# silencht/SG-SLAM

Measured on AMD Instinct MI355X. Metric: tracked frames/sec (640x480 RGB-D), higher is better.
Workload: dtype u8/f32(bf16x3 matrix products)/f64

## Files before the change

### include/sgx_debug.h

```cpp
#ifndef SGX_DEBUG_H
#define SGX_DEBUG_H
#include "sgx.h"
#ifdef __cplusplus
extern "C" {
#endif

int sgx_orb_debug_level_geometry(const sgx_orb *h, int level, int32_t *w, int32_t *hgt, int32_t *stride);
int sgx_orb_debug_set_unfused_pyramid(int on);
int sgx_orb_debug_read_level(sgx_orb *h, int frame, int level, uint8_t *dst );
int sgx_orb_debug_read_candidates(sgx_orb *h, int frame, int level, int32_t *x, int32_t *y, int32_t *score, int cap, int *n);
int sgx_debug_flow_affine_batch_dev(int batch, int cap, const sgx_keypoint *d_keys, const int32_t *d_n, const float *d_A, const float *d_shift, const float *d_boxes,
                                    int max_boxes, float *d_prev_xy, void *stream);
int sgx_pose_opt_debug_set_threads(int threads_per_frame);
int sgx_ba_debug_last_plan(int32_t plan[4]);
int sgx_ba_debug_set_init(int mode);
int sgx_ba_debug_set_jobs(int host);
int sgx_ba_debug_set_solver(int mode);
int sgx_det_debug_read_blob(sgx_det *h, const char *blob_name, int image, float *dst, int cap, int *n);
int sgx_flow_debug_read_level(sgx_flow *h, int slot, int frame, int level, uint8_t *img);
int sgx_flow_debug_level_size(const sgx_flow *h, int level, int32_t *w, int32_t *hgt);
int sgx_pnp_debug_betas(int which, const double *L, const double *rho, double *betas);
int sgx_debug_corun_bf16(int blocks, int iters, int launches, void *stream);
int sgx_det_debug_detection_output(sgx_det *h, const float *loc, const float *conf, int batch, sgx_det_result *results);
int sgx_det_debug_continued(sgx_det *h, int *count);
int sgx_det_debug_set_fusion(int on);
int sgx_det_debug_set_irb(int on);
int sgx_det_debug_set_block_fusion(int on);
int sgx_det_debug_set_gemm(int mode);
int sgx_det_debug_set_legacy_kernels(int on);
int sgx_det_debug_time_ops(sgx_det *h, const uint8_t *d_img, int pitch, int batch, int reps, float *ms, int cap, int *nops);
int sgx_det_debug_run_step(sgx_det *h, const uint8_t *d_img, int pitch, int batch, int step, int reps, void *stream);
int sgx_orb_debug_run_octree(sgx_orb *h, int level, const uint32_t *packed, int n, uint32_t *out_sel, int cap, int *nsel);

#ifdef __cplusplus
}
#endif
#endif
```

### sg_slam_amd/capi.py

```python
import ctypes as C
import numpy as np

KP_DTYPE = np.dtype([('x', 'f4'), ('y', 'f4'), ('size', 'f4'), ('angle', 'f4'), ('response', 'f4'),
                     ('octave', 'i4'), ('class_id', 'i4')])


class SgxError(RuntimeError):
    pass


class Camera(C.Structure):
    _fields_ = [('fx', C.c_float), ('fy', C.c_float), ('cx', C.c_float), ('cy', C.c_float), ('bf', C.c_float),
                ('min_x', C.c_float), ('max_x', C.c_float), ('min_y', C.c_float), ('max_y', C.c_float)]


class BaProblem(C.Structure):
    _fields_ = [('n_poses', C.c_int32), ('n_points', C.c_int32), ('n_edges', C.c_int32), ('poses', C.c_void_p), ('pose_fixed', C.c_void_p),
                ('points', C.c_void_p), ('edge_pose', C.c_void_p), ('edge_point', C.c_void_p), ('edge_obs', C.c_void_p), ('edge_info', C.c_void_p)]


class BaStats(C.Structure):
    _fields_ = [('iterations_first', C.c_int32), ('iterations_second', C.c_int32), ('free_poses', C.c_int32), ('reserved', C.c_int32),
                ('chi2_first', C.c_double), ('chi2_second', C.c_double)]


SGX_DET_MAX = 100


class Detection(C.Structure):
    _fields_ = [(k, C.c_float) for k in ('label', 'score', 'xmin', 'ymin', 'xmax', 'ymax')]


class Object2D(C.Structure):
    _fields_ = [('id', C.c_int32)] + [(k, C.c_float) for k in ('prob', 'x', 'y', 'w', 'h')]


class DetResult(C.Structure):
    _fields_ = [('n_raw', C.c_int32), ('raw', Detection * SGX_DET_MAX), ('n_objects', C.c_int32), ('objects', Object2D * SGX_DET_MAX),
                ('have_dynamic_for_mapping', C.c_int32), ('have_dynamic_for_rm_feature', C.c_int32),
                ('n_map_boxes', C.c_int32), ('map_boxes', Object2D * SGX_DET_MAX), ('n_rm_boxes', C.c_int32), ('rm_boxes', Object2D * SGX_DET_MAX)]


class FlowConfig(C.Structure):
    _fields_ = [('width', C.c_int32), ('height', C.c_int32), ('max_batch', C.c_int32), ('win_size', C.c_int32), ('max_level', C.c_int32),
                ('max_count', C.c_int32), ('epsilon', C.c_double)]


class TrackerConfig(C.Structure):
    _fields_ = [('streams', C.c_int32), ('width', C.c_int32), ('height', C.c_int32), ('nfeatures', C.c_int32), ('scale_factor', C.c_float), ('nlevels', C.c_int32),
                ('ini_th_fast', C.c_int32), ('min_th_fast', C.c_int32), ('cam', Camera), ('depth_map_factor', C.c_float), ('th_projection', C.c_float),
                ('local_map', C.c_int32), ('dynamic_mask', C.c_int32), ('max_boxes', C.c_int32), ('pipelined', C.c_int32)]


class OrbConfig(C.Structure):
    _fields_ = [('nfeatures', C.c_int32), ('scale_factor', C.c_float), ('nlevels', C.c_int32),
                ('ini_th_fast', C.c_int32), ('min_th_fast', C.c_int32), ('width', C.c_int32),
                ('height', C.c_int32), ('max_batch', C.c_int32)]


SYMBOLS = [
    'sgx_version', 'sgx_status_string', 'sgx_orb_create', 'sgx_orb_destroy', 'sgx_orb_keypoint_capacity', 'sgx_orb_get_tables',
    'sgx_orb_extract_batch_dev', 'sgx_orb_extract', 'sgx_orb_last_status', 'sgx_profile_enable', 'sgx_profile_num_classes', 'sgx_profile_class_name',
    'sgx_profile_read', 'sgx_match_project_frame_batch_dev', 'sgx_match_project_frame', 'sgx_match_project_local_batch_dev',
    'sgx_match_project_local', 'sgx_frame_stereo_from_rgbd_batch_dev', 'sgx_frame_unproject_batch_dev', 'sgx_frame_make_map_points_batch_dev',
    'sgx_frame_merge_matches_batch_dev', 'sgx_pose_optimization_batch_dev', 'sgx_pose_optimization', 'sgx_frame_motion_model_batch_dev',
    'sgx_local_bundle_adjustment', 'sgx_bundle_adjustment', 'sgx_det_create', 'sgx_det_destroy', 'sgx_det_info', 'sgx_det_detect',
    'sgx_det_detect_batch_dev', 'sgx_det_forward_batch_dev', 'sgx_frame_compact_keys_batch_dev', 'sgx_frame_gray_from_color_batch_dev',
    'sgx_det_gemm_mode', 'sgx_det_plan_step', 'sgx_dynamic_mask_batch_dev', 'sgx_tracker_create', 'sgx_tracker_destroy',
    'sgx_tracker_keypoint_capacity', 'sgx_tracker_record_bytes', 'sgx_tracker_set_initial_pose', 'sgx_tracker_step_dev', 'sgx_tracker_host_buffers',
    'sgx_tracker_step_host', 'sgx_tracker_wait_inputs', 'sgx_tracker_sync', 'sgx_tracker_read', 'sgx_tracker_snapshot_pose_dev',
    'sgx_tracker_snapshot_boxes_dev', 'sgx_tracker_pack_records_dev', 'sgx_tracker_frame_dev', 'sgx_tracker_extractor', 'sgx_flow_create',
    'sgx_dist_unique_id', 'sgx_dist_create', 'sgx_dist_destroy', 'sgx_dist_world', 'sgx_dist_gather_records',
    'sgx_flow_destroy', 'sgx_flow_reset', 'sgx_flow_levels', 'sgx_flow_lk_batch_dev', 'sgx_flow_lk', 'sgx_fundamental_ransac_batch_dev',
    'sgx_find_fundamental_mat', 'sgx_hamming_matrix', 'sgx_hamming_matrix_dev', 'sgx_match_search_for_triangulation', 'sgx_match_search_by_bow',
    'sgx_match_search_by_bow_kf', 'sgx_match_fuse_search', 'sgx_match_project_keyframe', 'sgx_match_fuse_search_sim3',
    'sgx_triangulate_new_map_points', 'sgx_mappoint_update_normal_and_depth', 'sgx_mappoint_distinctive_descriptors', 'sgx_sim3_solver_create',
    'sgx_sim3_solver_set_ransac_parameters', 'sgx_sim3_solver_iterate', 'sgx_sim3_solver_get_estimate', 'sgx_sim3_solver_destroy',
    'sgx_match_search_for_initialization', 'sgx_voc_load', 'sgx_voc_create', 'sgx_voc_info', 'sgx_voc_destroy', 'sgx_voc_transform',
    'sgx_voc_transform_batch_dev', 'sgx_voc_score', 'sgx_match_project_sim3', 'sgx_match_search_by_sim3', 'sgx_optimize_sim3',
    'sgx_optimize_essential_graph', 'sgx_correct_map_points', 'sgx_undistort_points', 'sgx_frame_undistort_stereo_rgbd_batch_dev', 'sgx_frame_image_bounds',
    'sgx_tracker_set_distortion', 'sgx_tracker_frame_keys_un_dev', 'sgx_pnp_solver_create', 'sgx_pnp_solver_set_ransac_parameters', 'sgx_pnp_solver_iterate',
    'sgx_pnp_solver_get_estimate', 'sgx_pnp_solver_destroy', 'sgx_pnp_batch_create', 'sgx_pnp_batch_set_dev', 'sgx_pnp_batch_iterate_dev', 'sgx_pnp_batch_destroy',
]
TAP_SYMBOLS = [
    'sgx_orb_debug_level_geometry', 'sgx_orb_debug_set_unfused_pyramid', 'sgx_orb_debug_read_level', 'sgx_orb_debug_read_candidates',
    'sgx_orb_debug_run_octree', 'sgx_pose_opt_debug_set_threads', 'sgx_ba_debug_set_solver', 'sgx_ba_debug_set_jobs', 'sgx_ba_debug_set_init', 'sgx_ba_debug_last_plan', 'sgx_det_debug_read_blob',
    'sgx_det_debug_detection_output', 'sgx_det_debug_continued', 'sgx_debug_flow_affine_batch_dev', 'sgx_det_debug_set_fusion', 'sgx_det_debug_set_legacy_kernels',
    'sgx_det_debug_set_block_fusion', 'sgx_det_debug_set_irb', 'sgx_det_debug_set_gemm', 'sgx_det_debug_time_ops', 'sgx_det_debug_run_step', 'sgx_flow_debug_read_level',
    'sgx_flow_debug_level_size', 'sgx_debug_corun_bf16', 'sgx_pnp_debug_betas',
]


def _vp(x):
    if x is None:
        return None
    if isinstance(x, int):
        return C.c_void_p(x)
    if hasattr(x, 'data_ptr'):
        return C.c_void_p(x.data_ptr())
    return x.ctypes.data_as(C.c_void_p)


class SgxLib:
    def __init__(self, path):
        self.path = path
        self.dll = C.CDLL(path)
        d = self.dll
        d.sgx_version.restype = C.c_char_p
        d.sgx_status_string.restype = C.c_char_p
        d.sgx_status_string.argtypes = [C.c_int]
        d.sgx_orb_create.argtypes = [C.POINTER(OrbConfig), C.POINTER(C.c_void_p)]
        d.sgx_orb_destroy.argtypes = [C.c_void_p]
        d.sgx_orb_destroy.restype = None
        d.sgx_orb_keypoint_capacity.argtypes = [C.c_void_p]
        d.sgx_orb_get_tables.argtypes = [C.c_void_p] + [C.c_void_p] * 5
        d.sgx_orb_extract_batch_dev.argtypes = [C.c_void_p, C.c_void_p, C.c_int, C.c_int, C.c_void_p, C.c_void_p,
                                                C.c_void_p, C.c_int, C.c_void_p]
        d.sgx_orb_extract.argtypes = [C.c_void_p, C.c_void_p, C.c_int, C.c_void_p, C.c_void_p, C.c_int, C.POINTER(C.c_int)]
        d.sgx_orb_last_status.argtypes = [C.c_void_p, C.c_void_p]

        d.sgx_profile_enable.argtypes = [C.c_int]
        d.sgx_profile_class_name.restype = C.c_char_p
        d.sgx_profile_class_name.argtypes = [C.c_int]
        d.sgx_profile_read.argtypes = [C.c_void_p, C.c_void_p, C.c_int]

        vp = C.c_void_p
        d.sgx_match_project_frame_batch_dev.argtypes = [C.c_int, C.c_int] + [vp] * 13 + [C.POINTER(Camera), vp, C.c_int, C.c_float, C.c_int, C.c_int, vp, vp, vp]
        d.sgx_match_project_frame.argtypes = [C.c_int] + [vp] * 4 + [C.c_int] + [vp] * 7 + [C.POINTER(Camera), vp, C.c_int, C.c_float, C.c_int, C.c_int, vp, vp]
        d.sgx_frame_stereo_from_rgbd_batch_dev.argtypes = [C.c_int, C.c_int, vp, vp, vp, C.c_int, C.c_int, C.c_float, C.c_float, vp, vp, vp]
        d.sgx_frame_unproject_batch_dev.argtypes = [C.c_int, C.c_int, vp, vp, vp, vp, C.POINTER(Camera), vp, vp, vp]
        d.sgx_pose_optimization_batch_dev.argtypes = [C.c_int, C.c_int, vp, vp, vp, vp, vp, vp, C.c_int, vp, C.c_int, C.POINTER(Camera), vp, vp, vp, vp]
        d.sgx_pose_optimization.argtypes = [C.c_int, vp, vp, vp, vp, vp, C.c_int, C.POINTER(Camera), vp, vp, vp]
        d.sgx_frame_motion_model_batch_dev.argtypes = [C.c_int, vp, vp, vp, vp, vp]
        d.sgx_local_bundle_adjustment.argtypes = [C.POINTER(BaProblem), C.POINTER(Camera), vp, vp, C.POINTER(BaStats)]
        d.sgx_bundle_adjustment.argtypes = [C.POINTER(BaProblem), C.POINTER(Camera), C.c_int, vp, C.c_int, C.POINTER(BaStats)]
        d.sgx_det_create.argtypes = [C.c_char_p, vp, C.c_size_t, C.c_int, C.c_int, C.c_int, C.c_float, C.c_float, C.POINTER(vp)]
        d.sgx_det_destroy.argtypes = [vp]; d.sgx_det_destroy.restype = None
        d.sgx_det_info.argtypes = [vp, C.POINTER(C.c_int32), C.POINTER(C.c_int32), C.POINTER(C.c_int32), C.POINTER(C.c_double)]
        d.sgx_det_detect.argtypes = [vp, vp, C.c_int, C.c_int, C.POINTER(DetResult)]
        d.sgx_det_detect_batch_dev.argtypes = [vp, vp, C.c_int, C.c_int, vp, vp, vp, C.c_int, vp, vp]
        d.sgx_det_forward_batch_dev.argtypes = [vp, vp, C.c_int, C.c_int, C.POINTER(vp), C.POINTER(vp), vp]
        d.sgx_det_gemm_mode.argtypes = [vp]
        d.sgx_tracker_create.argtypes = [C.POINTER(TrackerConfig), vp, C.POINTER(vp)]
        d.sgx_tracker_destroy.argtypes = [vp]; d.sgx_tracker_destroy.restype = None
        d.sgx_tracker_keypoint_capacity.argtypes = [vp]
        d.sgx_tracker_record_bytes.argtypes = [vp]
        d.sgx_tracker_set_initial_pose.argtypes = [vp, vp]
        d.sgx_tracker_step_dev.argtypes = [vp, vp, C.c_int, vp, vp, C.c_int, vp]
        d.sgx_tracker_host_buffers.argtypes = [vp, C.c_int, C.POINTER(vp), C.POINTER(C.c_int), C.POINTER(vp)]
        d.sgx_tracker_step_host.argtypes = [vp, C.c_int, C.c_int]
        d.sgx_tracker_sync.argtypes = [vp]
        d.sgx_tracker_wait_inputs.argtypes = [vp, C.c_int]
        d.sgx_tracker_read.argtypes = [vp] * 10
        d.sgx_tracker_snapshot_pose_dev.argtypes = [vp, vp]
        d.sgx_tracker_snapshot_boxes_dev.argtypes = [vp, C.c_int, vp, vp]
        d.sgx_tracker_pack_records_dev.argtypes = [vp, vp, vp]
        d.sgx_dist_unique_id.argtypes = [vp]
        d.sgx_dist_create.argtypes = [vp, C.c_int, C.c_int, C.POINTER(vp)]
        d.sgx_dist_destroy.argtypes = [vp]; d.sgx_dist_destroy.restype = None
        d.sgx_dist_world.argtypes = [vp, C.POINTER(C.c_int32), C.POINTER(C.c_int32)]
        d.sgx_dist_gather_records.argtypes = [vp, vp, C.c_size_t, vp, C.c_int, vp]
        d.sgx_tracker_frame_dev.argtypes = [vp] + [C.POINTER(vp)] * 6
        d.sgx_tracker_extractor.argtypes = [vp]; d.sgx_tracker_extractor.restype = vp
        d.sgx_det_plan_step.argtypes = [vp, C.c_int, C.c_char_p, C.c_int]
        d.sgx_dynamic_mask_batch_dev.argtypes = [C.c_int, C.c_int, vp, vp, vp, vp, vp, vp, C.c_int, vp, vp]
        d.sgx_frame_gray_from_color_batch_dev.argtypes = [C.c_int, C.c_int, C.c_int, vp, C.c_int, C.c_int, C.c_int, vp, C.c_int, vp]
        d.sgx_frame_compact_keys_batch_dev.argtypes = [C.c_int, C.c_int, vp, vp, vp, vp, vp, C.c_int, vp, vp, vp, vp]
        d.sgx_match_project_local.argtypes = [C.c_int] + [vp] * 5 + [C.c_int] + [vp] * 7 + [C.POINTER(Camera), vp, C.c_int, C.c_float, C.c_float, C.c_float, C.c_float, vp, vp, vp]
        d.sgx_match_project_local_batch_dev.argtypes = [C.c_int, C.c_int] + [vp] * 6 + [C.c_int] + [vp] * 8 + [C.POINTER(Camera), vp, C.c_int, C.c_float, C.c_float, C.c_float, C.c_float, vp, vp, vp, vp]
        d.sgx_undistort_points.argtypes = [C.c_int, vp, vp, vp, C.c_int, vp]
        d.sgx_frame_undistort_stereo_rgbd_batch_dev.argtypes = [C.c_int, C.c_int, vp, vp, vp, C.c_int, C.POINTER(Camera), vp, C.c_int, C.c_int, C.c_float, vp, vp, vp, vp]
        d.sgx_frame_image_bounds.argtypes = [C.c_int, C.c_int, vp, vp, C.c_int, C.POINTER(Camera)]
        d.sgx_tracker_set_distortion.argtypes = [vp, vp, C.c_int, C.POINTER(Camera)]
        d.sgx_tracker_frame_keys_un_dev.argtypes = [vp, C.POINTER(vp)]
        d.sgx_frame_make_map_points_batch_dev.argtypes = [C.c_int, C.c_int, C.c_int] + [vp] * 7 + [C.c_int] + [vp] * 7
        d.sgx_frame_merge_matches_batch_dev.argtypes = [C.c_int, C.c_int] + [vp] * 10
        d.sgx_flow_create.argtypes = [C.POINTER(FlowConfig), C.POINTER(vp)]
        d.sgx_flow_destroy.argtypes = [vp]; d.sgx_flow_destroy.restype = None
        d.sgx_flow_reset.argtypes = [vp]
        d.sgx_flow_levels.argtypes = [vp]
        d.sgx_flow_lk_batch_dev.argtypes = [vp, vp, C.c_int, C.c_int, vp, vp, C.c_int, vp, vp, C.POINTER(C.c_int32), vp]
        d.sgx_flow_lk.argtypes = [vp, vp, vp, C.c_int, vp, C.c_int, vp, vp]
        d.sgx_fundamental_ransac_batch_dev.argtypes = [C.c_int, C.c_int] + [vp] * 6 + [C.c_int, C.c_double, C.c_double, vp, vp, vp, vp]
        d.sgx_find_fundamental_mat.argtypes = [vp, vp, C.c_int, C.c_double, C.c_double, vp, vp, vp]
        d.sgx_hamming_matrix.argtypes = [vp, C.c_int, vp, C.c_int, vp]
        d.sgx_optimize_essential_graph.argtypes = [C.c_int, vp, vp, C.c_int, vp, vp, vp, C.c_int, C.c_int, vp, vp]
        d.sgx_correct_map_points.argtypes = [C.c_int, vp, vp, C.c_int, vp, vp, vp]
        d.sgx_optimize_sim3.argtypes = [C.c_int] + [vp] * 9 + [C.c_float, C.c_int, vp, vp, vp]
        d.sgx_match_project_keyframe.argtypes = [C.c_int] + [vp] * 4 + [C.c_int] + [vp] * 6 + [C.POINTER(Camera), vp, C.c_int, C.c_float, C.c_float, C.c_int, C.c_int, vp, vp]
        d.sgx_match_search_by_bow.argtypes = [C.c_int] + [vp] * 4 + [C.c_int] + [vp] * 3 + [C.c_float, C.c_int, vp, vp]
        d.sgx_match_fuse_search_sim3.argtypes = [C.c_int, vp, vp, vp, C.c_int] + [vp] * 6 + [vp, vp, C.c_int, C.c_float, C.c_float, vp, vp, vp]
        d.sgx_match_project_sim3.argtypes = [C.c_int, vp, vp, vp, vp, C.c_int] + [vp] * 6 + [vp, vp, C.c_int, C.c_float, C.c_int, vp, vp]
        d.sgx_match_search_by_sim3.argtypes = ([C.c_int] + [vp] * 8) * 2 + [vp, vp, C.c_int, C.c_float, C.c_float, vp, vp, C.c_float, vp, vp]
        d.sgx_match_search_for_initialization.argtypes = [C.c_int, vp, vp, C.c_int, vp, vp, vp, C.c_int, C.c_float, C.c_int, vp, vp, vp]
        d.sgx_sim3_solver_create.argtypes = [C.c_int] + [vp] * 6 + [C.c_int, C.c_uint, vp]
        d.sgx_sim3_solver_set_ransac_parameters.argtypes = [vp, C.c_double, C.c_int, C.c_int]
        d.sgx_sim3_solver_iterate.argtypes = [vp, C.c_int] + [vp] * 7
        d.sgx_sim3_solver_get_estimate.argtypes = [vp] * 5
        d.sgx_sim3_solver_destroy.argtypes = [vp]; d.sgx_sim3_solver_destroy.restype = None
        d.sgx_pnp_solver_create.argtypes = [C.c_int] + [vp] * 4 + [C.c_uint, vp]
        d.sgx_pnp_solver_set_ransac_parameters.argtypes = [vp, C.c_double, C.c_int, C.c_int, C.c_int, C.c_float, C.c_float]
        d.sgx_pnp_solver_iterate.argtypes = [vp, C.c_int] + [vp] * 7
        d.sgx_pnp_solver_get_estimate.argtypes = [vp] * 6
        d.sgx_pnp_solver_destroy.argtypes = [vp]; d.sgx_pnp_solver_destroy.restype = None
        d.sgx_pnp_batch_create.argtypes = [C.c_int, C.c_int, vp]
        d.sgx_pnp_batch_set_dev.argtypes = [vp, C.c_int] + [vp] * 8
        d.sgx_pnp_batch_iterate_dev.argtypes = [vp, C.c_int, vp, C.c_int, vp, vp, vp, vp]
        d.sgx_pnp_batch_destroy.argtypes = [vp]; d.sgx_pnp_batch_destroy.restype = None
        d.sgx_mappoint_update_normal_and_depth.argtypes = [C.c_int] + [vp] * 6 + [C.c_int, vp, vp, vp]
        d.sgx_mappoint_distinctive_descriptors.argtypes = [C.c_int, vp, vp, vp, vp]
        d.sgx_triangulate_new_map_points.argtypes = [C.c_int, vp] + [C.c_int] + [vp] * 5 + [C.c_int] + [vp] * 5 + [vp, vp, vp, C.c_int, vp, vp, vp]
        d.sgx_voc_load.argtypes = [C.c_char_p, vp]
        d.sgx_voc_create.argtypes = [C.c_int] * 5 + [vp] * 5
        d.sgx_voc_info.argtypes = [vp] * 7
        d.sgx_voc_destroy.argtypes = [vp]; d.sgx_voc_destroy.restype = None
        d.sgx_voc_transform.argtypes = [vp, C.c_int, vp, C.c_int, vp, vp, vp, vp, vp]
        d.sgx_voc_transform_batch_dev.argtypes = [vp, vp, C.c_size_t, vp, C.c_int, C.c_int, C.c_int, vp, vp, vp, vp]
        d.sgx_voc_score.argtypes = [vp, C.c_int, vp, vp, C.c_int, vp, vp, vp]
        d.sgx_match_search_by_bow_kf.argtypes = [C.c_int] + [vp] * 4 + [C.c_int] + [vp] * 4 + [C.c_float, C.c_int, vp, vp]
        d.sgx_match_fuse_search.argtypes = [C.c_int] + [vp] * 4 + [C.c_int] + [vp] * 6 + [C.POINTER(Camera), vp, vp, C.c_int, C.c_float, C.c_float, vp, vp, vp]
        d.sgx_hamming_matrix_dev.argtypes = [vp, C.c_int, vp, C.c_int, vp, vp]
        d.sgx_match_search_for_triangulation.argtypes = [C.c_int] + [vp] * 6 + [C.c_int] + [vp] * 6 + [vp, C.POINTER(Camera), vp, vp, C.c_int, C.c_int, C.c_int, vp, vp]

        self.has_taps = hasattr(d, 'sgx_det_debug_read_blob')
        if self.has_taps:
            d.sgx_orb_debug_level_geometry.argtypes = [C.c_void_p, C.c_int] + [C.POINTER(C.c_int32)] * 3
            d.sgx_orb_debug_read_level.argtypes = [C.c_void_p, C.c_int, C.c_int, C.c_void_p]
            d.sgx_orb_debug_read_candidates.argtypes = [C.c_void_p, C.c_int, C.c_int, C.c_void_p, C.c_void_p, C.c_void_p, C.c_int, C.POINTER(C.c_int)]
            d.sgx_orb_debug_run_octree.argtypes = [C.c_void_p, C.c_int, C.c_void_p, C.c_int, C.c_void_p, C.c_int, C.POINTER(C.c_int)]
            d.sgx_orb_debug_set_unfused_pyramid.argtypes = [C.c_int]
            d.sgx_pose_opt_debug_set_threads.argtypes = [C.c_int]
            d.sgx_ba_debug_set_solver.argtypes = [C.c_int]
            d.sgx_ba_debug_set_jobs.argtypes = [C.c_int]
            d.sgx_ba_debug_set_init.argtypes = [C.c_int]
            d.sgx_ba_debug_last_plan.argtypes = [C.c_void_p]
            d.sgx_det_debug_detection_output.argtypes = [vp, vp, vp, C.c_int, C.POINTER(DetResult)]
            d.sgx_det_debug_continued.argtypes = [vp, C.POINTER(C.c_int)]
            d.sgx_det_debug_read_blob.argtypes = [vp, C.c_char_p, C.c_int, vp, C.c_int, C.POINTER(C.c_int)]
            for nm in ('fusion', 'legacy_kernels', 'block_fusion', 'irb', 'gemm'):
                getattr(d, 'sgx_det_debug_set_' + nm).argtypes = [C.c_int]
            d.sgx_det_debug_time_ops.argtypes = [vp, vp, C.c_int, C.c_int, C.c_int, vp, C.c_int, C.POINTER(C.c_int)]
            d.sgx_det_debug_run_step.argtypes = [vp, vp, C.c_int, C.c_int, C.c_int, C.c_int, vp]
            d.sgx_debug_flow_affine_batch_dev.argtypes = [C.c_int, C.c_int, vp, vp, vp, vp, vp, C.c_int, vp, vp]
            d.sgx_flow_debug_read_level.argtypes = [vp, C.c_int, C.c_int, C.c_int, vp]
            d.sgx_debug_corun_bf16.argtypes = [C.c_int, C.c_int, C.c_int, vp]
            d.sgx_pnp_debug_betas.argtypes = [C.c_int, vp, vp, vp]
            d.sgx_flow_debug_level_size.argtypes = [vp, C.c_int, C.POINTER(C.c_int32), C.POINTER(C.c_int32)]

    def tap(self, name):
        if not self.has_taps:
            raise SgxError(f'{name}: {self.path} is the product build and has no test taps; use tests/taps/libsgx_taps.so (make -C sg_slam_amd/csrc taps)')
        return getattr(self.dll, name)

    def version(self):
        return self.dll.sgx_version().decode()

    def check(self, rc, what=''):
        if rc != 0:
            raise SgxError(f'{what}: {self.dll.sgx_status_string(rc).decode()} ({rc})')

    def profile_enable(self, on=True):
        self.check(self.dll.sgx_profile_enable(int(on)))

    def profile_read(self, reset=True):
        n = self.dll.sgx_profile_num_classes()
        ms = np.zeros(n, 'f4'); cnt = np.zeros(n, 'i4')
        self.check(self.dll.sgx_profile_read(_vp(ms), _vp(cnt), int(reset)), 'sgx_profile_read')
        return {self.dll.sgx_profile_class_name(k).decode(): (float(ms[k]), int(cnt[k])) for k in range(n)}
```

### sg_slam_amd/csrc/sgx_flow.cpp

```cpp
#include "sgx_flow_kernels.h"
#include "sgx_prof.h"
#include "sgx_stage.h"
#include "../../include/sgx.h"
#ifdef SGX_DEBUG_TAPS
#include "../../include/sgx_debug.h"
#endif
#include <stdio.h>
#include <stdlib.h>
#include <string.h>
#include <new>
#include <vector>


struct sgx_flow {
    sgx_flow_config cfg;
    SgxLkGeom g;
    uint8_t *img[2] = { nullptr, nullptr };
    int cur = 0;
    int prev_batch = 0;
};

extern "C" int sgx_flow_create(const sgx_flow_config *cfg, sgx_flow **out)
{
    if (!cfg || !out) return SGX_ERR_INVALID;
    *out = nullptr;
    if (cfg->width < 1 || cfg->height < 1 || cfg->max_batch < 1 || cfg->max_count < 0 || !(cfg->epsilon >= 0)) return SGX_ERR_INVALID;
    if (cfg->win_size != SGX_LK_WIN || cfg->max_level < 0 || cfg->max_level >= SGX_LK_MAXL) return SGX_ERR_UNSUPPORTED;
    if (cfg->width <= 1 || cfg->height <= 1) return SGX_ERR_UNSUPPORTED;
    { const unsigned long long qw = (unsigned long long)((cfg->width + 3) >> 2); if (qw * qw * (unsigned long long)cfg->height >= (1ull << 32)) return SGX_ERR_UNSUPPORTED; }
    sgx_flow *h = new (std::nothrow) sgx_flow();
    if (!h) return SGX_ERR_NOMEM;
    h->cfg = *cfg;
    SgxLkGeom &g = h->g;
    memset(&g, 0, sizeof g);
    int w = cfg->width, hh = cfg->height; unsigned io = 0;
    for (int l = 0;; l++) {
        g.w[l] = w; g.h[l] = hh; g.pitch[l] = (w + 3) & ~3; g.ioff[l] = io;
        io += (unsigned)g.pitch[l] * (unsigned)hh;
        g.nl = l + 1;
        if (l == cfg->max_level) break;
        const int nw = (w + 1) / 2, nh = (hh + 1) / 2;
        if (nw <= cfg->win_size || nh <= cfg->win_size) break;
        w = nw; hh = nh;
    }
    g.img_stride = (io + 15u + 64u) & ~15u;
    for (int s = 0; s < 2; s++)
        if (hipMalloc((void **)&h->img[s], (size_t)g.img_stride * cfg->max_batch) != hipSuccess) { sgx_flow_destroy(h); return SGX_ERR_NOMEM; }
    *out = h;
    return SGX_OK;
}

extern "C" void sgx_flow_destroy(sgx_flow *h)
{
    if (!h) return;
    for (int s = 0; s < 2; s++) if (h->img[s]) (void)hipFree(h->img[s]);
    delete h;
}

extern "C" int sgx_flow_reset(sgx_flow *h) { if (!h) return SGX_ERR_INVALID; h->prev_batch = 0; return SGX_OK; }
extern "C" int sgx_flow_levels(const sgx_flow *h) { return h ? h->g.nl : SGX_ERR_INVALID; }

static int build_pyramid(sgx_flow *h, int slot, const uint8_t *d_gray, int pitch, int batch, sgx_stream_t st)
{
    const SgxLkGeom &g = h->g;
    uint8_t *base = h->img[slot];
    sgx_prof_begin(SGX_K_LK_PYR, st);
    auto magic = [](int d) -> unsigned { return d <= 1 ? 0u : (unsigned)((0x100000000ull + (unsigned)d - 1) / (unsigned)d); };
    SGX_LAUNCH(k_lk_copy, dim3(((g.pitch[0] >> 2) * g.h[0] + 255) / 256, batch), dim3(256), st, d_gray, g.w[0], g.h[0], pitch, base, g.pitch[0], g.img_stride, magic(g.pitch[0] >> 2));
    for (int l = 1; l < g.nl; l++)
        SGX_LAUNCH(k_lk_pyrdown, dim3(((g.pitch[l] >> 2) * g.h[l] + 255) / 256, batch), dim3(256), st, (const uint8_t *)(base + g.ioff[l - 1]), g.w[l - 1], g.h[l - 1], g.pitch[l - 1],
                   g.img_stride, base + g.ioff[l], g.w[l], g.h[l], g.pitch[l], g.img_stride, magic(g.pitch[l] >> 2));
    sgx_prof_end(SGX_K_LK_PYR, st);
    SGX_CHECK_HIP(hipGetLastError());
    return SGX_OK;
}

static int track(sgx_flow *h, int cur_slot, int prev_slot, int batch, const sgx_keypoint *d_keys, const int32_t *d_n, int cap, float *d_prev_xy, uint8_t *d_status, sgx_stream_t st)
{
    SgxLkArgs A;
    A.cur_img = h->img[cur_slot]; A.prev_img = h->img[prev_slot];
    A.keys = (const uint8_t *)d_keys; A.n = d_n; A.cap = cap; A.prev_xy = d_prev_xy; A.status = d_status;
    A.max_count = h->cfg.max_count > 100 ? 100 : h->cfg.max_count;
    double eps = h->cfg.epsilon > 10. ? 10. : h->cfg.epsilon;
    A.eps2 = eps * eps; A.min_eig = (float)1e-4;
    sgx_prof_begin(SGX_K_LK_TRACK, st);
    static const int kpw = sgx_getenv("SGX_LK_KPW") ? atoi(sgx_getenv("SGX_LK_KPW")) : 2;
    A.batch = batch; A.kblocks = (cap + 4 * kpw - 1) / (4 * kpw);
#ifdef SGX_DEBUG_TAPS
    if (kpw == 4) { auto kfn = k_lk_trackN<4>; SGX_LAUNCH(kfn, dim3((unsigned)A.kblocks * (unsigned)batch), dim3(256), st, h->g, A); }
    else if (kpw != 2) { A.kblocks = (cap + 3) / 4; SGX_LAUNCH(k_lk_track, dim3((unsigned)A.kblocks * (unsigned)batch), dim3(256), st, h->g, A); }
    else
#endif
    { auto kfn = k_lk_trackN<2>; SGX_LAUNCH(kfn, dim3((unsigned)A.kblocks * (unsigned)batch), dim3(256), st, h->g, A); }
    sgx_prof_end(SGX_K_LK_TRACK, st);
    SGX_CHECK_HIP(hipGetLastError());
    return SGX_OK;
}

extern "C" int sgx_flow_lk_batch_dev(sgx_flow *h, const uint8_t *d_gray, int pitch, int batch, const sgx_keypoint *d_keys, const int32_t *d_n, int cap,
                                     float *d_prev_xy, uint8_t *d_status, int32_t *have_prev, void *stream)
{
    if (!h || !d_gray || batch < 1 || batch > h->cfg.max_batch || pitch < h->cfg.width) return SGX_ERR_INVALID;
    if ((pitch & 3) || ((uintptr_t)d_gray & 3)) return SGX_ERR_INVALID;
    sgx_stream_t st = (sgx_stream_t)stream;
    const int cur = h->cur, prev = cur ^ 1;
    const bool tracked = h->prev_batch == batch;
    if (tracked && (!d_keys || !d_n || !d_prev_xy || cap < 1)) return SGX_ERR_INVALID;
    int rc = build_pyramid(h, cur, d_gray, pitch, batch, st);
    if (rc != SGX_OK) return rc;
    if (tracked) { rc = track(h, cur, prev, batch, d_keys, d_n, cap, d_prev_xy, d_status, st); if (rc != SGX_OK) return rc; }
    if (have_prev) *have_prev = tracked ? 1 : 0;
    h->cur = prev; h->prev_batch = batch;
    return SGX_OK;
}

extern "C" int sgx_flow_lk(sgx_flow *h, const uint8_t *gray_from, const uint8_t *gray_to, int stride, const float *pts, int n, float *next_pts, uint8_t *status)
{
    if (!h || !gray_from || !gray_to || stride < h->cfg.width || n < 0 || (n > 0 && (!pts || !next_pts))) return SGX_ERR_INVALID;
    if (n == 0) return SGX_OK;
    const int W = h->cfg.width, H = h->cfg.height, P = (W + 3) & ~3;
    std::vector<uint8_t> pack((size_t)P * H * 2, 0);
    for (int y = 0; y < H; y++) { memcpy(&pack[(size_t)y * P], gray_to + (size_t)y * stride, (size_t)W); memcpy(&pack[(size_t)(H + y) * P], gray_from + (size_t)y * stride, (size_t)W); }
    std::vector<sgx_keypoint> kp((size_t)n);
    for (int i = 0; i < n; i++) { memset(&kp[(size_t)i], 0, sizeof(sgx_keypoint)); kp[(size_t)i].x = pts[2 * i]; kp[(size_t)i].y = pts[2 * i + 1]; }
    SgxStaged dI, dK, dN, dO, dS;
    int rc;
    if ((rc = dI.put(0, pack.data(), pack.size())) != SGX_OK || (rc = dK.put(1, kp.data(), kp.size() * sizeof(sgx_keypoint))) != SGX_OK ||
        (rc = dN.put(2, &n, sizeof n)) != SGX_OK || (rc = dO.put(3, nullptr, (size_t)n * 8)) != SGX_OK || (rc = dS.put(4, nullptr, (size_t)n)) != SGX_OK) return rc;
    const int keep_cur = h->cur, keep_prev = h->prev_batch;
    if ((rc = build_pyramid(h, 1, (const uint8_t *)dI.p, P, 1, 0)) != SGX_OK) return rc;
    if ((rc = build_pyramid(h, 0, (const uint8_t *)dI.p + (size_t)P * H, P, 1, 0)) != SGX_OK) return rc;
    if ((rc = track(h, 0, 1, 1, (const sgx_keypoint *)dK.p, (const int32_t *)dN.p, n, (float *)dO.p, (uint8_t *)dS.p, 0)) != SGX_OK) return rc;
    SGX_CHECK_HIP(hipMemcpy(next_pts, dO.p, (size_t)n * 8, hipMemcpyDeviceToHost));
    if (status) SGX_CHECK_HIP(hipMemcpy(status, dS.p, (size_t)n, hipMemcpyDeviceToHost));
    h->cur = keep_cur; h->prev_batch = 0; (void)keep_prev;
    return SGX_OK;
}

SGX_TAP int sgx_flow_debug_read_level(sgx_flow *h, int slot, int frame, int level, uint8_t *img )
{
    if (!h || slot < 0 || slot > 1 || frame < 0 || frame >= h->cfg.max_batch || level < 0 || level >= h->g.nl) return SGX_ERR_INVALID;
    const SgxLkGeom &g = h->g;
    SGX_CHECK_HIP(hipDeviceSynchronize());
    if (!img) return SGX_ERR_INVALID;
    {
        std::vector<uint8_t> t((size_t)g.pitch[level] * g.h[level]);
        SGX_CHECK_HIP(hipMemcpy(t.data(), h->img[slot] + (size_t)frame * g.img_stride + g.ioff[level], t.size(), hipMemcpyDeviceToHost));
        for (int y = 0; y < g.h[level]; y++) memcpy(img + (size_t)y * g.w[level], &t[(size_t)y * g.pitch[level]], (size_t)g.w[level]);
    }
    return SGX_OK;
}
SGX_TAP int sgx_flow_debug_level_size(const sgx_flow *h, int level, int32_t *w, int32_t *hh)
{
    if (!h || level < 0 || level >= h->g.nl || !w || !hh) return SGX_ERR_INVALID;
    *w = h->g.w[level]; *hh = h->g.h[level];
    return SGX_OK;
}

#if defined(SGX_DEBUG_TAPS) && !defined(SGX_EMU)
typedef float sgx_dbg_f16v __attribute__((ext_vector_type(16)));
typedef __bf16 sgx_dbg_bf8 __attribute__((ext_vector_type(8)));
SGX_KERNEL_OCC(256, 2) k_dbg_corun_bf16(float *o, int iters)
{
    const uint32_t x = threadIdx.x * 2654435761u + blockIdx.x, y = x ^ 0x9e3779b9u;
    sgx_dbg_f16v acc = {0}; sgx_dbg_bf8 a, b;
    for (int i = 0; i < 8; i++) { a[i] = (__bf16)(float)((x >> i) & 7); b[i] = (__bf16)(float)((y >> i) & 3); }
    for (int i = 0; i < iters; i++) acc = __builtin_amdgcn_mfma_f32_32x32x16_bf16(a, b, acc, 0, 0, 0);
    float s = 0.f; for (int i = 0; i < 16; i++) s += acc[i];
    o[(blockIdx.x & 1023) * 256 + threadIdx.x] = s;
}
#endif
SGX_TAP int sgx_debug_corun_bf16(int blocks, int iters, int launches, void *stream)
{
#if defined(SGX_DEBUG_TAPS) && !defined(SGX_EMU)
    static float *sink = nullptr;
    if (blocks < 1 || iters < 1 || launches < 1) return SGX_ERR_INVALID;
    if (!sink) SGX_CHECK_HIP(hipMalloc((void **)&sink, 1024 * 256 * sizeof(float)));
    for (int l = 0; l < launches; l++) SGX_LAUNCH(k_dbg_corun_bf16, dim3((unsigned)blocks), dim3(256), (sgx_stream_t)stream, sink, iters);
    SGX_CHECK_HIP(hipGetLastError());
    return SGX_OK;
#else
    (void)blocks; (void)iters; (void)launches; (void)stream;
    return SGX_ERR_UNSUPPORTED;
#endif
}

extern "C" int sgx_fundamental_ransac_batch_dev(int batch, int cap, const sgx_keypoint *d_keys, const int32_t *d_n, const float *d_prev_xy,
                                                const int32_t *d_pre_have_dynamic, const float *d_pre_boxes, const int32_t *d_pre_nboxes, int max_boxes,
                                                double threshold, double confidence, double *d_F, int32_t *d_ok, int32_t *d_stats, void *stream)
{
    if (batch < 1 || cap < 1 || !d_keys || !d_n || !d_prev_xy || !d_F || !d_ok || max_boxes < 0) return SGX_ERR_INVALID;
    if (cap > SGX_FM_MAXPTS) return SGX_ERR_UNSUPPORTED;
    SgxFmArgs A;
    A.keys = (const uint8_t *)d_keys; A.n = d_n; A.cap = cap; A.prev_xy = d_prev_xy;
    A.pre_have = d_pre_have_dynamic; A.pre_boxes = d_pre_boxes; A.pre_nboxes = d_pre_nboxes; A.max_boxes = max_boxes;
    if (threshold <= 0) threshold = 3;
    if (confidence < DBL_EPSILON || confidence > 1 - DBL_EPSILON) confidence = 0.99;
    A.threshold = threshold; A.confidence = confidence; A.max_iters = 1000;
    A.F = d_F; A.ok = d_ok; A.stats = d_stats;
    const size_t lds = (size_t)cap * 16 + 1024 + (((size_t)cap + 15) & ~(size_t)15);
    sgx_prof_begin(SGX_K_FM_RANSAC, (sgx_stream_t)stream);
    SGX_LAUNCH_DYN(k_fm_ransac, dim3(batch), dim3(256), lds, (sgx_stream_t)stream, A);
    sgx_prof_end(SGX_K_FM_RANSAC, (sgx_stream_t)stream);
    SGX_CHECK_HIP(hipGetLastError());
    return SGX_OK;
}

extern "C" int sgx_find_fundamental_mat(const float *pts1, const float *pts2, int n, double threshold, double confidence, double *F, int32_t *ok, int32_t *stats)
{
    if (n < 0 || (n > 0 && (!pts1 || !pts2)) || !F || !ok) return SGX_ERR_INVALID;
    if (n > SGX_FM_MAXPTS) return SGX_ERR_UNSUPPORTED;
    const int cap = n > 0 ? n : 1;
    std::vector<sgx_keypoint> kp((size_t)cap);
    memset(kp.data(), 0, kp.size() * sizeof(sgx_keypoint));
    for (int i = 0; i < n; i++) { kp[(size_t)i].x = pts1[2 * i]; kp[(size_t)i].y = pts1[2 * i + 1]; }
    SgxStaged dK, dN, dP, dF, dO, dS;
    int rc;
    if ((rc = dK.put(0, kp.data(), kp.size() * sizeof(sgx_keypoint))) != SGX_OK || (rc = dN.put(1, &n, sizeof n)) != SGX_OK ||
        (rc = dP.put(2, n ? pts2 : nullptr, (size_t)cap * 8)) != SGX_OK || (rc = dF.put(3, nullptr, 72)) != SGX_OK || (rc = dO.put(4, nullptr, 4)) != SGX_OK ||
        (rc = dS.put(5, nullptr, 16)) != SGX_OK) return rc;
    rc = sgx_fundamental_ransac_batch_dev(1, cap, (const sgx_keypoint *)dK.p, (const int32_t *)dN.p, (const float *)dP.p, nullptr, nullptr, nullptr, 0, threshold, confidence,
                                          (double *)dF.p, (int32_t *)dO.p, (int32_t *)dS.p, nullptr);
    if (rc != SGX_OK) return rc;
    SGX_CHECK_HIP(hipMemcpy(F, dF.p, 72, hipMemcpyDeviceToHost));
    SGX_CHECK_HIP(hipMemcpy(ok, dO.p, 4, hipMemcpyDeviceToHost));
    if (stats) SGX_CHECK_HIP(hipMemcpy(stats, dS.p, 16, hipMemcpyDeviceToHost));
    return SGX_OK;
}
```

### sg_slam_amd/csrc/sgx_flow_kernels.h

```cpp
#pragma once
#include "sgx_rt.h"
#include "sgx_block.h"
#include <float.h>
#include <math.h>

#define SGX_LK_MAXL 4
#define SGX_LK_WIN 21
#define SGX_LK_TILE_PITCH 36
struct SgxLkGeom {
    int nl;
    int w[SGX_LK_MAXL], h[SGX_LK_MAXL], pitch[SGX_LK_MAXL];
    unsigned ioff[SGX_LK_MAXL];
    unsigned img_stride;
};

SGX_DEV int sgx_reflect101(int p, int len)
{
    if (len == 1) return 0;
    while (p < 0 || p >= len) { if (p < 0) p = -p; else p = 2 * len - 2 - p; }
    return p;
}
SGX_DEV int sgx_floor_f(float v) { return (int)floorf(v); }
SGX_DEV float sgx_i64_to_f32(long long v)
{
    const long long hi = v >> 24; const int lo = (int)(v - (hi << 24));
    return (float)(int)hi * 16777216.0f + (float)lo;
}

SGX_DEV unsigned sgx_lk_udiv(unsigned n, unsigned m)
{
#ifndef SGX_EMU
    return m ? __umulhi(n, m) : n;
#else
    return m ? (unsigned)(((unsigned long long)n * m) >> 32) : n;
#endif
}
SGX_KERNEL(256) k_lk_copy(const uint8_t *src, int w, int h, int spitch, uint8_t *dst, int dpitch, unsigned dstride, unsigned qw_magic)
{
    SGX_THREADS_BEGIN(tid)
    const int f = (int)blockIdx.y, qw = dpitch >> 2, q = (int)blockIdx.x * 256 + tid;
    if (q < qw * h) {
        const int y = (int)sgx_lk_udiv((unsigned)q, qw_magic), x = (q - y * qw) * 4;
        const uint8_t *s = src + ((size_t)f * h + y) * spitch;
        uint32_t v;
        if (x + 4 <= w) v = *(const uint32_t *)(s + x);
        else { v = 0; for (int i = 0; x + i < w; i++) v |= (uint32_t)s[x + i] << (8 * i); }
        *(uint32_t *)(dst + (size_t)f * dstride + (size_t)y * dpitch + x) = v;
    }
    SGX_THREADS_END
}

SGX_KERNEL(256) k_lk_pyrdown(const uint8_t *src, int sw, int sh, int spitch, unsigned sstride, uint8_t *dst, int dw, int dh, int dpitch, unsigned dstride, unsigned qw_magic)
{
    SGX_THREADS_BEGIN(tid)
    const int f = (int)blockIdx.y, qw = dpitch >> 2, q = (int)blockIdx.x * 256 + tid;
    if (q < qw * dh) {
        const int y = (int)sgx_lk_udiv((unsigned)q, qw_magic), X = (q - y * qw) * 4;
        const uint8_t *S = src + (size_t)f * sstride;
        int acc[4] = { 0, 0, 0, 0 };
        const bool fast = X >= 2 && 2 * X + 11 < spitch && 2 * X + 8 <= sw - 1;
#pragma unroll
        for (int k = 0; k < 5; k++) {
            const int wk = k == 0 || k == 4 ? 1 : k == 2 ? 6 : 4;
            const uint8_t *row = S + (size_t)sgx_reflect101(2 * y - 2 + k, sh) * spitch;
            int p[11];
            if (fast) {
                const uint32_t *r4 = (const uint32_t *)(row + 2 * X - 4);
                const uint32_t a = r4[0], b = r4[1], c = r4[2], d = r4[3];
                p[0] = (a >> 16) & 255; p[1] = a >> 24;
                p[2] = b & 255; p[3] = (b >> 8) & 255; p[4] = (b >> 16) & 255; p[5] = b >> 24;
                p[6] = c & 255; p[7] = (c >> 8) & 255; p[8] = (c >> 16) & 255; p[9] = c >> 24;
                p[10] = d & 255;
            } else {
#pragma unroll
                for (int i = 0; i < 11; i++) p[i] = row[sgx_reflect101(2 * X - 2 + i, sw)];
            }
#pragma unroll
            for (int o = 0; o < 4; o++) acc[o] += wk * (p[2 * o + 2] * 6 + (p[2 * o + 1] + p[2 * o + 3]) * 4 + p[2 * o] + p[2 * o + 4]);
        }
        uint32_t out = 0;
#pragma unroll
        for (int o = 0; o < 4; o++) out |= (uint32_t)((acc[o] + 128) >> 8) << (8 * o);
        *(uint32_t *)(dst + (size_t)f * dstride + (size_t)y * dpitch + X) = out;
    }
    SGX_THREADS_END
}

struct SgxLkWeights { int w00, w01, w10, w11; };
SGX_DEV SgxLkWeights sgx_lk_weights(float a, float b)
{
    SgxLkWeights k;
    k.w00 = sgx_cvround((1.f - a) * (1.f - b) * (float)(1 << 14));
    k.w01 = sgx_cvround(a * (1.f - b) * (float)(1 << 14));
    k.w10 = sgx_cvround((1.f - a) * b * (float)(1 << 14));
    k.w11 = (1 << 14) - k.w00 - k.w01 - k.w10;
    return k;
}
#define SGX_LK_DESCALE(x, n) (((x) + (1 << ((n) - 1))) >> (n))

struct SgxLkStep { float dx, dy; };
SGX_DEV SgxLkStep sgx_lk_step(float A11, float A12, float A22, float D, long long sb1, long long sb2)
{
    const float FLT_SCALE = 1.f / (1 << 20);
    const float b1 = sgx_i64_to_f32(sb1) * FLT_SCALE, b2 = sgx_i64_to_f32(sb2) * FLT_SCALE;
    SgxLkStep s;
    s.dx = (A12 * b2 - A22 * b1) * D;
    s.dy = (A12 * b1 - A11 * b2) * D;
    return s;
}

struct SgxLkArgs {
    const uint8_t *cur_img, *prev_img;
    const uint8_t *keys; const int *n; int cap;
    float *prev_xy; uint8_t *status;
    int max_count; double eps2; float min_eig;
    int batch, kblocks;
};
SGX_DEV void sgx_lk_decode_block(int i, int batch, int kblocks, int &f, int &kb)
{
    const int full = (batch / 8) * 8;
    if (i < full * kblocks) { const int x = i & 7, j = i >> 3; kb = j % kblocks; f = x + 8 * (j / kblocks); }
    else { const int j = i - full * kblocks; f = full + j / kblocks; kb = j % kblocks; }
}

#ifdef SGX_EMU
static inline int sgx_lk_px(const uint8_t *I, int w, int h, int pitch, int x, int y) { return I[(size_t)sgx_reflect101(y, h) * pitch + sgx_reflect101(x, w)]; }
static void sgx_lk_track_point(const SgxLkGeom &g, const uint8_t *I0, const uint8_t *J0, float kx, float ky, int max_count, double eps2, float min_eig,
                               float *ox, float *oy, uint8_t *ost)
{
    const int W = SGX_LK_WIN; const float half = (W - 1) * 0.5f, FLT_SCALE = 1.f / (1 << 20);
    float outx = 0.f, outy = 0.f; uint8_t status = 1;
    static thread_local short Iw[SGX_LK_WIN * SGX_LK_WIN], dIw[SGX_LK_WIN * SGX_LK_WIN * 2];
    for (int level = g.nl - 1; level >= 0; level--) {
        const int w = g.w[level], h = g.h[level], pitch = g.pitch[level];
        const uint8_t *I = I0 + g.ioff[level], *J = J0 + g.ioff[level];
        const float sc = 1.0f / (float)(1 << level);
        float prevx = kx * sc, prevy = ky * sc, nextx, nexty;
        if (level == g.nl - 1) { nextx = prevx; nexty = prevy; } else { nextx = outx * 2.f; nexty = outy * 2.f; }
        outx = nextx; outy = nexty;
        prevx -= half; prevy -= half;
        const int ipx = sgx_floor_f(prevx), ipy = sgx_floor_f(prevy);
        if (ipx < -W || ipx >= w || ipy < -W || ipy >= h) { if (level == 0) status = 0; continue; }
        SgxLkWeights k = sgx_lk_weights(prevx - ipx, prevy - ipy);
        long long s11 = 0, s12 = 0, s22 = 0;
        for (int y = 0; y < W; y++) for (int x = 0; x < W; x++) {
            int pv[4], dx[4], dy[4];
            for (int c = 0; c < 4; c++) {
                const int gx = ipx + x + (c & 1), gy = ipy + y + (c >> 1);
                pv[c] = sgx_lk_px(I, w, h, pitch, gx, gy);
                if (gx < 0 || gy < 0 || gx >= w || gy >= h) { dx[c] = dy[c] = 0; }
                else {
                    int t0[3], t1[3];
                    for (int q = 0; q < 3; q++) {
                        const int a = sgx_lk_px(I, w, h, pitch, gx - 1 + q, gy - 1), b = sgx_lk_px(I, w, h, pitch, gx - 1 + q, gy), cc = sgx_lk_px(I, w, h, pitch, gx - 1 + q, gy + 1);
                        t0[q] = (a + cc) * 3 + b * 10; t1[q] = cc - a;
                    }
                    dx[c] = t0[2] - t0[0]; dy[c] = (t1[0] + t1[2]) * 3 + t1[1] * 10;
                }
            }
            const int iv = SGX_LK_DESCALE(pv[0] * k.w00 + pv[1] * k.w01 + pv[2] * k.w10 + pv[3] * k.w11, 9);
            const int ix = SGX_LK_DESCALE(dx[0] * k.w00 + dx[1] * k.w01 + dx[2] * k.w10 + dx[3] * k.w11, 14);
            const int iy = SGX_LK_DESCALE(dy[0] * k.w00 + dy[1] * k.w01 + dy[2] * k.w10 + dy[3] * k.w11, 14);
            Iw[y * W + x] = (short)iv; dIw[(y * W + x) * 2] = (short)ix; dIw[(y * W + x) * 2 + 1] = (short)iy;
            s11 += (long long)ix * ix; s12 += (long long)ix * iy; s22 += (long long)iy * iy;
        }
        const float A11 = sgx_i64_to_f32(s11) * FLT_SCALE, A12 = sgx_i64_to_f32(s12) * FLT_SCALE, A22 = sgx_i64_to_f32(s22) * FLT_SCALE;
        float D = A11 * A22 - A12 * A12;
        const float minEig = (A22 + A11 - sqrtf((A11 - A22) * (A11 - A22) + 4.f * A12 * A12)) / (float)(2 * W * W);
        if (minEig < min_eig || D < FLT_EPSILON) { if (level == 0) status = 0; continue; }
        D = 1.f / D;
        nextx -= half; nexty -= half;
        float pdx = 0.f, pdy = 0.f;
        for (int j = 0; j < max_count; j++) {
            const int inx = sgx_floor_f(nextx), iny = sgx_floor_f(nexty);
            if (inx < -W || inx >= w || iny < -W || iny >= h) { if (level == 0) status = 0; break; }
            k = sgx_lk_weights(nextx - inx, nexty - iny);
            long long sb1 = 0, sb2 = 0;
            for (int y = 0; y < W; y++) for (int x = 0; x < W; x++) {
                int pv[4];
                for (int c = 0; c < 4; c++) pv[c] = sgx_lk_px(J, w, h, pitch, inx + x + (c & 1), iny + y + (c >> 1));
                const int diff = SGX_LK_DESCALE(pv[0] * k.w00 + pv[1] * k.w01 + pv[2] * k.w10 + pv[3] * k.w11, 9) - Iw[y * W + x];
                sb1 += (long long)diff * dIw[(y * W + x) * 2]; sb2 += (long long)diff * dIw[(y * W + x) * 2 + 1];
            }
            const SgxLkStep st = sgx_lk_step(A11, A12, A22, D, sb1, sb2);
            nextx += st.dx; nexty += st.dy;
            outx = nextx + half; outy = nexty + half;
            if ((double)st.dx * st.dx + (double)st.dy * st.dy <= eps2) break;
            if (j > 0 && fabs((double)(st.dx + pdx)) < 0.01 && fabs((double)(st.dy + pdy)) < 0.01) { outx -= st.dx * 0.5f; outy -= st.dy * 0.5f; break; }
            pdx = st.dx; pdy = st.dy;
        }
        if (status && level == 0) {
            const int ix = sgx_floor_f(outx - half), iy = sgx_floor_f(outy - half);
            if (ix < -W || ix >= w || iy < -W || iy >= h) status = 0;
        }
    }
    *ox = outx; *oy = outy; *ost = status;
}
SGX_KERNEL(256) k_lk_track(SgxLkGeom g, SgxLkArgs A)
{
    SGX_THREADS_BEGIN(tid)
    int f, kb;
    sgx_lk_decode_block((int)blockIdx.x, A.batch, A.kblocks, f, kb);
    const int kp = kb * 4 + (tid >> 6);
    if ((tid & 63) == 0 && kp < A.n[f] && kp < A.cap) {
        const float *kpt = (const float *)(A.keys + ((size_t)f * A.cap + kp) * 28);
        float ox, oy; uint8_t st;
        sgx_lk_track_point(g, A.cur_img + (size_t)f * g.img_stride, A.prev_img + (size_t)f * g.img_stride, kpt[0], kpt[1], A.max_count, A.eps2, A.min_eig, &ox, &oy, &st);
        A.prev_xy[2 * ((size_t)f * A.cap + kp)] = ox; A.prev_xy[2 * ((size_t)f * A.cap + kp) + 1] = oy;
        if (A.status) A.status[(size_t)f * A.cap + kp] = st;
    }
    SGX_THREADS_END
}
#else
SGX_DEV int sgx_wave_sum_i32(int v)
{
    v += __builtin_amdgcn_update_dpp(0, v, 0xB1, 0xF, 0xF, true);
    v += __builtin_amdgcn_update_dpp(0, v, 0x4E, 0xF, 0xF, true);
    v += __builtin_amdgcn_update_dpp(0, v, 0x124, 0xF, 0xF, true);
    v += __builtin_amdgcn_update_dpp(0, v, 0x128, 0xF, 0xF, true);
    v += __builtin_amdgcn_update_dpp(0, v, 0x142, 0xA, 0xF, false);
    v += __builtin_amdgcn_update_dpp(0, v, 0x143, 0xC, 0xF, false);
    return __builtin_amdgcn_readlane(v, 63);
}
SGX_DEV float sgx_wave_sum_f32(int v)
{
    const int lo = sgx_wave_sum_i32(v & 0xFFFF), hi = sgx_wave_sum_i32(v >> 16);
    return fmaf((float)hi, 65536.0f, (float)lo);
}
SGX_DEV int sgx_mul24(int a, int b) { return __mul24(a, b); }
SGX_DEV int sgx_reflect1(int p, int len) { p = p < 0 ? -p : p; p = p >= len ? 2 * len - 2 - p : p; return min(max(p, 0), len - 1); }

typedef short sgx_i16x2 __attribute__((ext_vector_type(2)));
typedef unsigned short sgx_u16x2 __attribute__((ext_vector_type(2)));
SGX_DEV sgx_i16x2 sgx_as_i16x2(uint32_t v) { return __builtin_bit_cast(sgx_i16x2, v); }
SGX_DEV uint32_t sgx_as_u32(sgx_i16x2 v) { return __builtin_bit_cast(uint32_t, v); }
#define SGX_LK_PAIR(hi, lo, a, b) sgx_as_i16x2(__builtin_amdgcn_perm((hi), (lo), (uint32_t)(a) | 0x0c00u | ((uint32_t)(b) << 16) | 0x0c000000u))
SGX_DEV sgx_i16x2 sgx_lk_next(sgx_i16x2 p, sgx_i16x2 q) { return sgx_as_i16x2(__builtin_amdgcn_alignbit(sgx_as_u32(q), sgx_as_u32(p), 16)); }
#if defined(SGX_LK_NODOT) && !defined(SGX_EMU)
SGX_DEV int sgx_lk_dot2_mad(sgx_i16x2 a, sgx_i16x2 b, int c)
{
    const uint32_t ua = __builtin_bit_cast(uint32_t, a), ub = __builtin_bit_cast(uint32_t, b);
    asm("v_mad_i32_i16 %0, %1, %2, %0 op_sel:[0,0,0,0]" : "+v"(c) : "v"(ua), "v"(ub));
    asm("v_mad_i32_i16 %0, %1, %2, %0 op_sel:[1,1,0,0]" : "+v"(c) : "v"(ua), "v"(ub));
    return c;
}
#define SGX_LK_DOT2(a, b, c) sgx_lk_dot2_mad((a), (b), (c))
#else
#define SGX_LK_DOT2(a, b, c) __builtin_amdgcn_sdot2((a), (b), (c), false)
#endif
SGX_DEV int sgx_lk_dot2_keep(sgx_i16x2 a, sgx_i16x2 b, int c) { return SGX_LK_DOT2(a, b, c); }

template <int PASSES>
SGX_DEV void sgx_lk_stage(uint32_t *tile, const uint8_t *img, int w, int h, int pitch, int ox, int oy, int rl, int cl)
{
    __builtin_amdgcn_fence(__ATOMIC_SEQ_CST, "wavefront"); __builtin_amdgcn_wave_barrier();
    const int gx = ox + 4 * cl;
    const bool inside = gx >= 0 && gx + 4 <= w;
    if (rl < 7) {
        uint32_t v[PASSES];
        if (inside) {
#pragma unroll
            for (int p = 0; p < PASSES; p++) v[p] = *(const uint32_t *)(img + (size_t)sgx_reflect1(oy + p * 7 + rl, h) * pitch + gx);
        } else {
            const int x0 = sgx_reflect1(gx, w), x1 = sgx_reflect1(gx + 1, w), x2 = sgx_reflect1(gx + 2, w), x3 = sgx_reflect1(gx + 3, w);
#pragma unroll
            for (int p = 0; p < PASSES; p++) {
                const uint8_t *src = img + (size_t)sgx_reflect1(oy + p * 7 + rl, h) * pitch;
                v[p] = (uint32_t)src[x0] | ((uint32_t)src[x1] << 8) | ((uint32_t)src[x2] << 16) | ((uint32_t)src[x3] << 24);
            }
        }
#pragma unroll
        for (int p = 0; p < PASSES; p++) tile[(p * 7 + rl) * (SGX_LK_TILE_PITCH / 4) + cl] = v[p];
    }
    __builtin_amdgcn_fence(__ATOMIC_SEQ_CST, "wavefront"); __builtin_amdgcn_wave_barrier();
}

#ifdef SGX_DEBUG_TAPS
SGX_KERNEL(256) k_lk_track(SgxLkGeom g, SgxLkArgs A)
{
    __shared__ uint32_t tiles[4][35 * SGX_LK_TILE_PITCH / 4 + 5];
    const int tid = (int)threadIdx.x, lane = tid & 63, wv = tid >> 6;
    int f, kb;
    sgx_lk_decode_block((int)blockIdx.x, A.batch, A.kblocks, f, kb);
    const int kp = kb * 4 + wv;
    if (kp >= A.n[f] || kp >= A.cap) return;
    uint32_t *tile = tiles[wv];
    const uint8_t *tile8 = (const uint8_t *)tile;
    const int W = SGX_LK_WIN; const float half = 10.0f, FLT_SCALE = 1.f / (1 << 20);
    const float *kpt = (const float *)(A.keys + ((size_t)f * A.cap + kp) * 28);
    const float kx = __builtin_bit_cast(float, __builtin_amdgcn_readfirstlane(__builtin_bit_cast(int, kpt[0])));
    const float ky = __builtin_bit_cast(float, __builtin_amdgcn_readfirstlane(__builtin_bit_cast(int, kpt[1])));
    const uint8_t *I0 = A.cur_img + (size_t)f * g.img_stride, *J0 = A.prev_img + (size_t)f * g.img_stride;
    const int r = lane / 3, s7 = (lane - 3 * r) * 7;
    const int rl = lane / 9, cl = lane - 9 * rl;
    const bool active = lane < 63;
    const int lane_off = active ? r * SGX_LK_TILE_PITCH + s7 : 0;
    float outx = 0.f, outy = 0.f; int status = 1;

    for (int level = g.nl - 1; level >= 0; level--) {
        const int w = g.w[level], h = g.h[level], pitch = g.pitch[level];
        const uint8_t *I = I0 + g.ioff[level], *J = J0 + g.ioff[level];
        const float sc = 1.0f / (float)(1 << level);
        float prevx = kx * sc, prevy = ky * sc, nextx, nexty;
        if (level == g.nl - 1) { nextx = prevx; nexty = prevy; } else { nextx = outx * 2.f; nexty = outy * 2.f; }
        outx = nextx; outy = nexty;
        prevx -= half; prevy -= half;
        const int ipx = sgx_floor_f(prevx), ipy = sgx_floor_f(prevy);
        if (ipx < -W || ipx >= w || ipy < -W || ipy >= h) { if (level == 0) status = 0; continue; }
        SgxLkWeights k = sgx_lk_weights(prevx - ipx, prevy - ipy);
        sgx_i16x2 W0 = sgx_as_i16x2((uint32_t)k.w00 | ((uint32_t)k.w01 << 16)), W1 = sgx_as_i16x2((uint32_t)k.w10 | ((uint32_t)k.w11 << 16));

        int ivb[7]; int ix[7], iy[7];
        int s11 = 0, s12 = 0, s22 = 0;
        {
            const int gy0 = ipy + r, gx0 = ipx + s7;
            sgx_i16x2 P[4][5];
            const bool direct = ipx >= 1 && ipx + 25 < w && ipy >= 1 && ipy + 22 < h;
            if (direct) {
                const uint8_t *gb = I + (size_t)(active ? gy0 - 1 : ipy) * pitch + (active ? gx0 - 1 : ipx);
#pragma unroll
                for (int j = 0; j < 4; j++) {
                    uint32_t q[3];
                    __builtin_memcpy(q, gb + (size_t)j * pitch, 12);
                    P[j][0] = SGX_LK_PAIR(q[0], q[0], 0, 1); P[j][1] = SGX_LK_PAIR(q[0], q[0], 2, 3);
                    P[j][2] = SGX_LK_PAIR(q[1], q[1], 0, 1); P[j][3] = SGX_LK_PAIR(q[1], q[1], 2, 3);
                    P[j][4] = SGX_LK_PAIR(q[2], q[2], 0, 1);
                }
            } else {
                const int tx = ((ipx - 1) >> 2) << 2, ty = ipy - 1;
                sgx_lk_stage<4>(tile, I, w, h, pitch, tx, ty, rl, cl);
                const uint8_t *tb = tile8 + lane_off + (ipx - 1 - tx);
#pragma unroll
                for (int j = 0; j < 4; j++) {
                    uint32_t q[3];
                    __builtin_memcpy(q, tb + j * SGX_LK_TILE_PITCH, 12);
                    P[j][0] = SGX_LK_PAIR(q[0], q[0], 0, 1); P[j][1] = SGX_LK_PAIR(q[0], q[0], 2, 3);
                    P[j][2] = SGX_LK_PAIR(q[1], q[1], 0, 1); P[j][3] = SGX_LK_PAIR(q[1], q[1], 2, 3);
                    P[j][4] = SGX_LK_PAIR(q[2], q[2], 0, 1);
                }
            }
            const sgx_i16x2 c3 = { 3, 3 }, c10 = { 10, 10 };
            const sgx_i16x2 Wd0 = active ? W0 : sgx_as_i16x2(0u), Wd1 = active ? W1 : sgx_as_i16x2(0u);
            sgx_i16x2 S0[5], S1[5], D0[5], D1[5];
#pragma unroll
            for (int q = 0; q < 5; q++) {
                S0[q] = (P[0][q] + P[2][q]) * c3 + P[1][q] * c10; D0[q] = P[2][q] - P[0][q];
                S1[q] = (P[1][q] + P[3][q]) * c3 + P[2][q] * c10; D1[q] = P[3][q] - P[1][q];
            }
            sgx_i16x2 xa[5], ya[5], xb[5], yb[5];
            const bool whole = ipx >= 0 && ipx + W < w && ipy >= 0 && ipy + W < h;
#pragma unroll
            for (int q = 0; q < 4; q++) {
                xa[q] = S0[q + 1] - S0[q]; ya[q] = (D0[q] + D0[q + 1]) * c3 + sgx_lk_next(D0[q], D0[q + 1]) * c10;
                xb[q] = S1[q + 1] - S1[q]; yb[q] = (D1[q] + D1[q + 1]) * c3 + sgx_lk_next(D1[q], D1[q + 1]) * c10;
            }
            if (!whole) {
                const bool rowa = gy0 >= 0 && gy0 < h, rowb = gy0 + 1 >= 0 && gy0 + 1 < h;
#pragma unroll
                for (int q = 0; q < 4; q++) {
                    const int x = gx0 + 2 * q;
                    const uint32_t m = ((x >= 0 && x < w) ? 0xFFFFu : 0u) | ((x + 1 >= 0 && x + 1 < w) ? 0xFFFF0000u : 0u);
                    const uint32_t ma = rowa ? m : 0u, mb = rowb ? m : 0u;
                    xa[q] = sgx_as_i16x2(sgx_as_u32(xa[q]) & ma); ya[q] = sgx_as_i16x2(sgx_as_u32(ya[q]) & ma);
                    xb[q] = sgx_as_i16x2(sgx_as_u32(xb[q]) & mb); yb[q] = sgx_as_i16x2(sgx_as_u32(yb[q]) & mb);
                }
            }
#pragma unroll
            for (int c = 0; c < 7; c++) {
                const sgx_i16x2 pxa = (c & 1) ? sgx_lk_next(xa[c >> 1], xa[(c >> 1) + 1]) : xa[c >> 1], pxb = (c & 1) ? sgx_lk_next(xb[c >> 1], xb[(c >> 1) + 1]) : xb[c >> 1];
                const sgx_i16x2 pya = (c & 1) ? sgx_lk_next(ya[c >> 1], ya[(c >> 1) + 1]) : ya[c >> 1], pyb = (c & 1) ? sgx_lk_next(yb[c >> 1], yb[(c >> 1) + 1]) : yb[c >> 1];
                const sgx_i16x2 pia = (c & 1) ? P[1][(c + 1) >> 1] : sgx_lk_next(P[1][c >> 1], P[1][(c >> 1) + 1]), pib = (c & 1) ? P[2][(c + 1) >> 1] : sgx_lk_next(P[2][c >> 1], P[2][(c >> 1) + 1]);
                const int v = SGX_LK_DOT2(pib, W1, SGX_LK_DOT2(pia, W0, 256)) >> 9;
                const int vx = SGX_LK_DOT2(pxb, Wd1, SGX_LK_DOT2(pxa, Wd0, 8192)) >> 14;
                const int vy = SGX_LK_DOT2(pyb, Wd1, SGX_LK_DOT2(pya, Wd0, 8192)) >> 14;
                ivb[c] = 256 - (v << 9); ix[c] = vx; iy[c] = vy;
                s11 += sgx_mul24(vx, vx); s12 += sgx_mul24(vx, vy); s22 += sgx_mul24(vy, vy);
            }
        }
        const float A11 = sgx_wave_sum_f32(s11) * FLT_SCALE, A12 = sgx_wave_sum_f32(s12) * FLT_SCALE, A22 = sgx_wave_sum_f32(s22) * FLT_SCALE;
        float D = A11 * A22 - A12 * A12;
        const float minEig = (A22 + A11 - sqrtf((A11 - A22) * (A11 - A22) + 4.f * A12 * A12)) / (float)(2 * W * W);
        if (minEig < A.min_eig || D < FLT_EPSILON) { if (level == 0) status = 0; continue; }
        D = 1.f / D;
        nextx -= half; nexty -= half;
        float pdx = 0.f, pdy = 0.f;
        int ox = 0, oy = 0; bool staged = false;
        for (int j = 0; j < A.max_count; j++) {
            const int inx = sgx_floor_f(nextx), iny = sgx_floor_f(nexty);
            if (inx < -W || inx >= w || iny < -W || iny >= h) { if (level == 0) status = 0; break; }
            k = sgx_lk_weights(nextx - inx, nexty - iny);
            W0 = sgx_as_i16x2((uint32_t)k.w00 | ((uint32_t)k.w01 << 16)); W1 = sgx_as_i16x2((uint32_t)k.w10 | ((uint32_t)k.w11 << 16));
            if (!staged || inx < ox || inx - ox > SGX_LK_TILE_PITCH - 22 || iny < oy || iny - oy > 35 - 22) {
                ox = ((inx - 5) >> 2) << 2; oy = iny - 6;
                sgx_lk_stage<5>(tile, J, w, h, pitch, ox, oy, rl, cl);
                staged = true;
            }
            int sb1 = 0, sb2 = 0;
            {
                const uint8_t *tb = tile8 + lane_off + (iny - oy) * SGX_LK_TILE_PITCH + (inx - ox);
                uint32_t a[2], b[2];
                __builtin_memcpy(a, tb, 8); __builtin_memcpy(b, tb + SGX_LK_TILE_PITCH, 8);
#pragma unroll
                for (int c = 0; c < 7; c++) {
                    const int diff = SGX_LK_DOT2(SGX_LK_PAIR(b[1], b[0], c, c + 1), W1, SGX_LK_DOT2(SGX_LK_PAIR(a[1], a[0], c, c + 1), W0, ivb[c])) >> 9;
                    sb1 += sgx_mul24(diff, ix[c]); sb2 += sgx_mul24(diff, iy[c]);
                }
            }
            const float b1 = sgx_wave_sum_f32(sb1) * FLT_SCALE, b2 = sgx_wave_sum_f32(sb2) * FLT_SCALE;
            const float dx = (A12 * b2 - A22 * b1) * D, dy = (A12 * b1 - A11 * b2) * D;
            nextx += dx; nexty += dy;
            outx = nextx + half; outy = nexty + half;
            if ((double)dx * dx + (double)dy * dy <= A.eps2) break;
            if (j > 0 && fabs((double)(dx + pdx)) < 0.01 && fabs((double)(dy + pdy)) < 0.01) { outx -= dx * 0.5f; outy -= dy * 0.5f; break; }
            pdx = dx; pdy = dy;
        }
        if (status && level == 0) {
            const int qx = sgx_floor_f(outx - half), qy = sgx_floor_f(outy - half);
            if (qx < -W || qx >= w || qy < -W || qy >= h) status = 0;
        }
    }
    if (lane == 0) {
        A.prev_xy[2 * ((size_t)f * A.cap + kp)] = outx; A.prev_xy[2 * ((size_t)f * A.cap + kp) + 1] = outy;
        if (A.status) A.status[(size_t)f * A.cap + kp] = (uint8_t)status;
    }
}
#endif
#endif

#ifndef SGX_EMU
SGX_DEV int sgx_row_sum_i32(int v)
{
    v += __builtin_amdgcn_update_dpp(v, v, 0xB1, 0xF, 0xF, true);
    v += __builtin_amdgcn_update_dpp(v, v, 0x4E, 0xF, 0xF, true);
    v += __builtin_amdgcn_update_dpp(v, v, 0x124, 0xF, 0xF, true);
    v += __builtin_amdgcn_update_dpp(v, v, 0x128, 0xF, 0xF, true);
    return v;
}
template <int LPK>
SGX_DEV float sgx_group_sum_f32(int v)
{
    int lo = sgx_row_sum_i32(v & 0xFFFF), hi = sgx_row_sum_i32(v >> 16);
    if (LPK == 32) { lo += __shfl_xor(lo, 16, 64); hi += __shfl_xor(hi, 16, 64); }
    return fmaf((float)hi, 65536.0f, (float)lo);
}

#define SGX_LK4_PITCH 32
template <int NROWS, int LPK>
SGX_DEV void sgx_lk_stage_row(uint32_t *tile, const uint8_t *img, int w, int h, int pitch, int ox, int oy, int l16)
{
    constexpr int RPP = LPK / 8, G = LPK == 16 ? 6 : 3;
    const int c = l16 & 7, rs = l16 >> 3, gx = ox + 4 * c;
    const bool inside = gx >= 0 && gx + 4 <= w;
    const int x0 = sgx_reflect1(gx, w), x1 = sgx_reflect1(gx + 1, w), x2 = sgx_reflect1(gx + 2, w), x3 = sgx_reflect1(gx + 3, w);
#pragma unroll 1
    for (int r0 = rs; r0 < NROWS; r0 += RPP * G) {
        uint32_t v[G];
#pragma unroll
        for (int p = 0; p < G; p++) {
            const uint8_t *src = img + (size_t)sgx_reflect1(oy + min(r0 + RPP * p, NROWS - 1), h) * pitch;
            if (inside) v[p] = *(const uint32_t *)(src + gx);
            else v[p] = (uint32_t)src[x0] | ((uint32_t)src[x1] << 8) | ((uint32_t)src[x2] << 16) | ((uint32_t)src[x3] << 24);
        }
#pragma unroll
        for (int p = 0; p < G; p++) { const int r = r0 + RPP * p; if (r < NROWS) tile[r * (SGX_LK4_PITCH / 4) + c] = v[p]; }
    }
}

SGX_DEV void sgx_lk_segment_setup(const sgx_i16x2 (&P)[4][5], sgx_i16x2 W0, sgx_i16x2 W1, bool whole, int gx0, int gy0, int w, int h,
                                  int (&ivb)[7], uint32_t (&ixy)[7], int &s11, int &s12, int &s22)
{
    const sgx_i16x2 c3 = { 3, 3 }, c10 = { 10, 10 };
    sgx_i16x2 S0[5], S1[5], D0[5], D1[5];
#pragma unroll
    for (int q = 0; q < 5; q++) {
        S0[q] = (P[0][q] + P[2][q]) * c3 + P[1][q] * c10; D0[q] = P[2][q] - P[0][q];
        S1[q] = (P[1][q] + P[3][q]) * c3 + P[2][q] * c10; D1[q] = P[3][q] - P[1][q];
    }
    sgx_i16x2 xa[5], ya[5], xb[5], yb[5];
#pragma unroll
    for (int q = 0; q < 4; q++) {
        xa[q] = S0[q + 1] - S0[q]; ya[q] = (D0[q] + D0[q + 1]) * c3 + sgx_lk_next(D0[q], D0[q + 1]) * c10;
        xb[q] = S1[q + 1] - S1[q]; yb[q] = (D1[q] + D1[q + 1]) * c3 + sgx_lk_next(D1[q], D1[q + 1]) * c10;
    }
    if (!whole) {
        const bool rowa = gy0 >= 0 && gy0 < h, rowb = gy0 + 1 >= 0 && gy0 + 1 < h;
#pragma unroll
        for (int q = 0; q < 4; q++) {
            const int x = gx0 + 2 * q;
            const uint32_t m = ((x >= 0 && x < w) ? 0xFFFFu : 0u) | ((x + 1 >= 0 && x + 1 < w) ? 0xFFFF0000u : 0u);
            const uint32_t ma = rowa ? m : 0u, mb = rowb ? m : 0u;
            xa[q] = sgx_as_i16x2(sgx_as_u32(xa[q]) & ma); ya[q] = sgx_as_i16x2(sgx_as_u32(ya[q]) & ma);
            xb[q] = sgx_as_i16x2(sgx_as_u32(xb[q]) & mb); yb[q] = sgx_as_i16x2(sgx_as_u32(yb[q]) & mb);
        }
    }
#pragma unroll
    for (int c = 0; c < 7; c++) {
        const sgx_i16x2 pxa = (c & 1) ? sgx_lk_next(xa[c >> 1], xa[(c >> 1) + 1]) : xa[c >> 1], pxb = (c & 1) ? sgx_lk_next(xb[c >> 1], xb[(c >> 1) + 1]) : xb[c >> 1];
        const sgx_i16x2 pya = (c & 1) ? sgx_lk_next(ya[c >> 1], ya[(c >> 1) + 1]) : ya[c >> 1], pyb = (c & 1) ? sgx_lk_next(yb[c >> 1], yb[(c >> 1) + 1]) : yb[c >> 1];
        const sgx_i16x2 pia = (c & 1) ? P[1][(c + 1) >> 1] : sgx_lk_next(P[1][c >> 1], P[1][(c >> 1) + 1]), pib = (c & 1) ? P[2][(c + 1) >> 1] : sgx_lk_next(P[2][c >> 1], P[2][(c >> 1) + 1]);
        const int v = SGX_LK_DOT2(pib, W1, SGX_LK_DOT2(pia, W0, 256)) >> 9;
        const int vx = SGX_LK_DOT2(pxb, W1, SGX_LK_DOT2(pxa, W0, 8192)) >> 14;
        const int vy = SGX_LK_DOT2(pyb, W1, SGX_LK_DOT2(pya, W0, 8192)) >> 14;
        ivb[c] = 256 - (v << 9); ixy[c] = ((uint32_t)vx & 0xFFFFu) | ((uint32_t)vy << 16);
        s11 += sgx_mul24(vx, vx); s12 += sgx_mul24(vx, vy); s22 += sgx_mul24(vy, vy);
    }
}
SGX_DEV int sgx_mad_lo16(int diff, uint32_t pair, int acc) { asm("v_mad_i32_i16 %0, %1, %2, %0 op_sel:[0,0,0,0]" : "+v"(acc) : "v"(diff), "v"(pair)); return acc; }
SGX_DEV int sgx_mad_hi16(int diff, uint32_t pair, int acc) { asm("v_mad_i32_i16 %0, %1, %2, %0 op_sel:[0,1,0,0]" : "+v"(acc) : "v"(diff), "v"(pair)); return acc; }

template <int KPW>
SGX_KERNEL_OCC(256, (KPW == 4 ? 3 : 5)) k_lk_trackN(SgxLkGeom g, SgxLkArgs A)
{
    constexpr int LPK = 64 / KPW, SPL = KPW;
    constexpr int TD = 36 * SGX_LK4_PITCH / 4 + 5;
    __shared__ uint32_t tiles[4 * KPW][TD];
    const int tid = (int)threadIdx.x, lane = tid & 63, wv = tid >> 6, row = lane / LPK, l16 = lane % LPK;
    int f, kb;
    sgx_lk_decode_block((int)blockIdx.x, A.batch, A.kblocks, f, kb);
    const int nkp = min(A.n[f], A.cap);
    if (kb * (4 * KPW) + wv * KPW >= nkp) return;
    const int kp = kb * (4 * KPW) + wv * KPW + row;
    const bool valid = kp < nkp;
    uint32_t *tile = tiles[wv * KPW + row];
    const uint8_t *tile8 = (const uint8_t *)tile;
    const int W = SGX_LK_WIN; const float half = 10.0f, FLT_SCALE = 1.f / (1 << 20);
    const float *kpt = (const float *)(A.keys + ((size_t)f * A.cap + (valid ? kp : 0)) * 28);
    const float kx = kpt[0], ky = kpt[1];
    const uint8_t *I0 = A.cur_img + (size_t)f * g.img_stride, *J0 = A.prev_img + (size_t)f * g.img_stride;
    int soff[SPL], srow[SPL], scol[SPL];
#pragma unroll
    for (int q = 0; q < SPL; q++) { const int si = min(l16 + LPK * q, 62); srow[q] = si / 3; scol[q] = (si - 3 * srow[q]) * 7; soff[q] = srow[q] * SGX_LK4_PITCH + scol[q]; }
    const bool idle3 = l16 == LPK - 1;
    float outx = 0.f, outy = 0.f; int status = 1;

    for (int level = g.nl - 1; level >= 0; level--) {
        const int w = g.w[level], h = g.h[level], pitch = g.pitch[level];
        const uint8_t *I = I0 + g.ioff[level], *J = J0 + g.ioff[level];
        const float sc = 1.0f / (float)(1 << level);
        float prevx = kx * sc, prevy = ky * sc, nextx, nexty;
        if (level == g.nl - 1) { nextx = prevx; nexty = prevy; } else { nextx = outx * 2.f; nexty = outy * 2.f; }
        outx = nextx; outy = nexty;
        prevx -= half; prevy -= half;
        const int ipx = sgx_floor_f(prevx), ipy = sgx_floor_f(prevy);
        bool act = valid;
        if (ipx < -W || ipx >= w || ipy < -W || ipy >= h) { if (level == 0) status = 0; act = false; }
        if (!__any(act)) continue;
        SgxLkWeights k = sgx_lk_weights(prevx - ipx, prevy - ipy);
        sgx_i16x2 W0 = sgx_as_i16x2((uint32_t)k.w00 | ((uint32_t)k.w01 << 16)), W1 = sgx_as_i16x2((uint32_t)k.w10 | ((uint32_t)k.w11 << 16));

        int ivb[SPL][7]; uint32_t ixy[SPL][7];
        int s11 = 0, s12 = 0, s22 = 0;
        {
            const bool direct = act && ipx >= 1 && ipx + 25 < w && ipy >= 1 && ipy + 22 < h;
            const bool whole = !__any(act && !(ipx >= 0 && ipx + W < w && ipy >= 0 && ipy + W < h));
            const int tx = ((ipx - 1) >> 2) << 2, ty = ipy - 1;
            if (__any(act && !direct)) {
                __builtin_amdgcn_fence(__ATOMIC_SEQ_CST, "wavefront"); __builtin_amdgcn_wave_barrier();
                if (act && !direct) sgx_lk_stage_row<28, LPK>(tile, I, w, h, pitch, tx, ty, l16);
                __builtin_amdgcn_fence(__ATOMIC_SEQ_CST, "wavefront"); __builtin_amdgcn_wave_barrier();
            }
#pragma unroll
            for (int q = 0; q < SPL; q++) {
                const int gy0 = ipy + srow[q], gx0 = ipx + scol[q];
                sgx_i16x2 P[4][5];
                if (direct) {
                    const uint8_t *gb = I + (size_t)(gy0 - 1) * pitch + (gx0 - 1);
#pragma unroll
                    for (int j = 0; j < 4; j++) {
                        uint32_t d[3];
                        __builtin_memcpy(d, gb + (size_t)j * pitch, 12);
                        P[j][0] = SGX_LK_PAIR(d[0], d[0], 0, 1); P[j][1] = SGX_LK_PAIR(d[0], d[0], 2, 3);
                        P[j][2] = SGX_LK_PAIR(d[1], d[1], 0, 1); P[j][3] = SGX_LK_PAIR(d[1], d[1], 2, 3);
                        P[j][4] = SGX_LK_PAIR(d[2], d[2], 0, 1);
                    }
                } else {
                    const uint8_t *tb = tile8 + soff[q] + (ipx - 1 - tx);
#pragma unroll
                    for (int j = 0; j < 4; j++) {
                        uint32_t d[3];
                        __builtin_memcpy(d, tb + j * SGX_LK4_PITCH, 12);
                        P[j][0] = SGX_LK_PAIR(d[0], d[0], 0, 1); P[j][1] = SGX_LK_PAIR(d[0], d[0], 2, 3);
                        P[j][2] = SGX_LK_PAIR(d[1], d[1], 0, 1); P[j][3] = SGX_LK_PAIR(d[1], d[1], 2, 3);
                        P[j][4] = SGX_LK_PAIR(d[2], d[2], 0, 1);
                    }
                }
                const bool on = act && !(q == SPL - 1 && idle3);
                const sgx_i16x2 Wq0 = on ? W0 : sgx_as_i16x2(0u), Wq1 = on ? W1 : sgx_as_i16x2(0u);
                sgx_lk_segment_setup(P, Wq0, Wq1, whole, gx0, gy0, w, h, ivb[q], ixy[q], s11, s12, s22);
                __builtin_amdgcn_sched_barrier(0);
            }
        }
        const float A11 = sgx_group_sum_f32<LPK>(s11) * FLT_SCALE, A12 = sgx_group_sum_f32<LPK>(s12) * FLT_SCALE, A22 = sgx_group_sum_f32<LPK>(s22) * FLT_SCALE;
        float D = A11 * A22 - A12 * A12;
        const float minEig = (A22 + A11 - sqrtf((A11 - A22) * (A11 - A22) + 4.f * A12 * A12)) / (float)(2 * W * W);
        if (act && (minEig < A.min_eig || D < FLT_EPSILON)) { if (level == 0) status = 0; act = false; }
        D = 1.f / D;
        nextx -= half; nexty -= half;
        float pdx = 0.f, pdy = 0.f;
        int ox = 0, oy = 0; bool staged = false;
        for (int j = 0; j < A.max_count; j++) {
            const int inx = sgx_floor_f(nextx), iny = sgx_floor_f(nexty);
            if (act && (inx < -W || inx >= w || iny < -W || iny >= h)) { if (level == 0) status = 0; act = false; }
            if (!__any(act)) break;
            k = sgx_lk_weights(nextx - inx, nexty - iny);
            W0 = sgx_as_i16x2((uint32_t)k.w00 | ((uint32_t)k.w01 << 16)); W1 = sgx_as_i16x2((uint32_t)k.w10 | ((uint32_t)k.w11 << 16));
            const bool need = act && (!staged || inx < ox || inx - ox > SGX_LK4_PITCH - 22 || iny < oy || iny - oy > 36 - 22);
            if (__any(need)) {
                __builtin_amdgcn_fence(__ATOMIC_SEQ_CST, "wavefront"); __builtin_amdgcn_wave_barrier();
                if (need) {
                    ox = ((inx - 3) >> 2) << 2; oy = iny - 7;
                    sgx_lk_stage_row<36, LPK>(tile, J, w, h, pitch, ox, oy, l16);
                    staged = true;
                }
                __builtin_amdgcn_fence(__ATOMIC_SEQ_CST, "wavefront"); __builtin_amdgcn_wave_barrier();
            }
            int sb1 = 0, sb2 = 0;
            if (act) {
                const uint8_t *tb0 = tile8 + (iny - oy) * SGX_LK4_PITCH + (inx - ox);
#pragma unroll
                for (int q = 0; q < SPL; q++) {
                    const uint8_t *tb = tb0 + soff[q];
                    uint32_t a[2], b[2];
                    __builtin_memcpy(a, tb, 8); __builtin_memcpy(b, tb + SGX_LK4_PITCH, 8);
#pragma unroll
                    for (int c = 0; c < 7; c++) {
                        const int diff = SGX_LK_DOT2(SGX_LK_PAIR(b[1], b[0], c, c + 1), W1, sgx_lk_dot2_keep(SGX_LK_PAIR(a[1], a[0], c, c + 1), W0, ivb[q][c])) >> 9;
                        sb1 = sgx_mad_lo16(diff, ixy[q][c], sb1); sb2 = sgx_mad_hi16(diff, ixy[q][c], sb2);
                    }
                }
            }
            const float b1 = sgx_group_sum_f32<LPK>(sb1) * FLT_SCALE, b2 = sgx_group_sum_f32<LPK>(sb2) * FLT_SCALE;
            if (act) {
                const float dx = (A12 * b2 - A22 * b1) * D, dy = (A12 * b1 - A11 * b2) * D;
                nextx += dx; nexty += dy;
                outx = nextx + half; outy = nexty + half;
                const float f2 = dx * dx + dy * dy, e2f = (float)A.eps2;
                bool conv = f2 <= e2f;
                if (__any(fabsf(f2 - e2f) <= 1e-5f * e2f)) { asm volatile("" ::: "memory"); conv = (double)dx * dx + (double)dy * dy <= A.eps2; }
                if (conv) act = false;
                else if (j > 0 && fabsf(dx + pdx) <= 0.01f && fabsf(dy + pdy) <= 0.01f) { outx -= dx * 0.5f; outy -= dy * 0.5f; act = false; }
                pdx = dx; pdy = dy;
            }
        }
        if (valid && status && level == 0) {
            const int qx = sgx_floor_f(outx - half), qy = sgx_floor_f(outy - half);
            if (qx < -W || qx >= w || qy < -W || qy >= h) status = 0;
        }
    }
    if (l16 == 0 && valid) {
        A.prev_xy[2 * ((size_t)f * A.cap + kp)] = outx; A.prev_xy[2 * ((size_t)f * A.cap + kp) + 1] = outy;
        if (A.status) A.status[(size_t)f * A.cap + kp] = (uint8_t)status;
    }
}
#else
template <int KPW>
SGX_KERNEL(256) k_lk_trackN(SgxLkGeom g, SgxLkArgs A)
{
    SGX_THREADS_BEGIN(tid)
    int f, kb;
    sgx_lk_decode_block((int)blockIdx.x, A.batch, A.kblocks, f, kb);
    const int kp = kb * (4 * KPW) + tid / (64 / KPW);
    if (tid % (64 / KPW) == 0 && kp < A.n[f] && kp < A.cap) {
        const float *kpt = (const float *)(A.keys + ((size_t)f * A.cap + kp) * 28);
        float ox, oy; uint8_t st;
        sgx_lk_track_point(g, A.cur_img + (size_t)f * g.img_stride, A.prev_img + (size_t)f * g.img_stride, kpt[0], kpt[1], A.max_count, A.eps2, A.min_eig, &ox, &oy, &st);
        A.prev_xy[2 * ((size_t)f * A.cap + kp)] = ox; A.prev_xy[2 * ((size_t)f * A.cap + kp) + 1] = oy;
        if (A.status) A.status[(size_t)f * A.cap + kp] = st;
    }
    SGX_THREADS_END
}
#endif

#define SGX_FM_CHUNK 32
#define SGX_FM_MAXPTS 2048

SGX_DEV int sgx_solve_cubic(const double *c, double *roots)
{
    double a0 = c[0], a1 = c[1], a2 = c[2], a3 = c[3];
    double x0 = 0., x1 = 0., x2 = 0.;
    int n = 0;
    if (a0 == 0) {
        if (a1 == 0) {
            if (a2 == 0) n = a3 == 0 ? -1 : 0;
            else { x0 = -a3 / a2; n = 1; }
        } else {
            double d = a2 * a2 - 4 * a1 * a3;
            if (d >= 0) {
                d = sqrt(d);
                double q1 = (-a2 + d) * 0.5, q2 = (a2 + d) * -0.5;
                if (fabs(q1) > fabs(q2)) { x0 = q1 / a1; x1 = a3 / q1; }
                else { x0 = q2 / a1; x1 = a3 / q2; }
                n = d > 0 ? 2 : 1;
            }
        }
    } else {
        a0 = 1. / a0; a1 *= a0; a2 *= a0; a3 *= a0;
        double Q = (a1 * a1 - 3 * a2) * (1. / 9);
        double R = (2 * a1 * a1 * a1 - 9 * a1 * a2 + 27 * a3) * (1. / 54);
        double Qcubed = Q * Q * Q;
        double d = Qcubed - R * R;
        if (d > 0) {
            double theta = acos(R / sqrt(Qcubed));
            double sqrtQ = sqrt(Q);
            double t0 = -2 * sqrtQ, t1 = theta * (1. / 3), t2 = a1 * (1. / 3);
            x0 = t0 * cos(t1) - t2;
            x1 = t0 * cos(t1 + (2. * 3.1415926535897932384626433832795 / 3)) - t2;
            x2 = t0 * cos(t1 + (4. * 3.1415926535897932384626433832795 / 3)) - t2;
            n = 3;
        } else if (d == 0) {
            if (R >= 0) { x0 = -2 * pow(R, 1. / 3) - a1 / 3; x1 = pow(R, 1. / 3) - a1 / 3; }
            else { x0 = 2 * pow(-R, 1. / 3) - a1 / 3; x1 = -pow(-R, 1. / 3) - a1 / 3; }
            x2 = 0;
            n = x0 == x1 ? 1 : 2;
            x1 = x0 == x1 ? 0 : x1;
        } else {
            double e;
            d = sqrt(-d);
            e = pow(d + fabs(R), 1. / 3);
            if (R > 0) e = -e;
            x0 = (e + Q / e) - a1 * (1. / 3);
            n = 1;
        }
    }
    roots[0] = x0; roots[1] = x1; roots[2] = x2;
    return n;
}

SGX_DEV int sgx_fm_run7point(const float *m1, const float *m2, double *M, double *fmatrix)
{
    double beta[7], f1[9], f2[9], c[4], r[3];
    for (int i = 0; i < 7; i++) {
        const double x0 = m1[2 * i], y0 = m1[2 * i + 1], x1 = m2[2 * i], y1 = m2[2 * i + 1];
        M[0 * 7 + i] = x1 * x0; M[1 * 7 + i] = x1 * y0; M[2 * 7 + i] = x1;
        M[3 * 7 + i] = y1 * x0; M[4 * 7 + i] = y1 * y0; M[5 * 7 + i] = y1;
        M[6 * 7 + i] = x0; M[7 * 7 + i] = y0; M[8 * 7 + i] = 1;
    }
    for (int k = 0; k < 7; k++) {
        double nrm = 0; for (int i = k; i < 9; i++) nrm += M[i * 7 + k] * M[i * 7 + k];
        nrm = sqrt(nrm);
        beta[k] = 0;
        if (nrm == 0) continue;
        M[k * 7 + k] += M[k * 7 + k] >= 0 ? nrm : -nrm;
        double vv = 0; for (int i = k; i < 9; i++) vv += M[i * 7 + k] * M[i * 7 + k];
        if (vv == 0) continue;
        beta[k] = 2. / vv;
        for (int j = k + 1; j < 7; j++) {
            double s = 0; for (int i = k; i < 9; i++) s += M[i * 7 + k] * M[i * 7 + j];
            s *= beta[k];
            for (int i = k; i < 9; i++) M[i * 7 + j] -= s * M[i * 7 + k];
        }
    }
    for (int i = 0; i < 9; i++) { f1[i] = i == 7; f2[i] = i == 8; }
    for (int k = 6; k >= 0; k--) {
        double s1 = 0, s2 = 0;
        for (int i = k; i < 9; i++) { s1 += M[i * 7 + k] * f1[i]; s2 += M[i * 7 + k] * f2[i]; }
        s1 *= beta[k]; s2 *= beta[k];
        for (int i = k; i < 9; i++) { f1[i] -= s1 * M[i * 7 + k]; f2[i] -= s2 * M[i * 7 + k]; }
    }
    for (int i = 0; i < 9; i++) f1[i] -= f2[i];
    double t0 = f2[4] * f2[8] - f2[5] * f2[7], t1 = f2[3] * f2[8] - f2[5] * f2[6], t2 = f2[3] * f2[7] - f2[4] * f2[6];
    c[3] = f2[0] * t0 - f2[1] * t1 + f2[2] * t2;
    c[2] = f1[0] * t0 - f1[1] * t1 + f1[2] * t2 -
           f1[3] * (f2[1] * f2[8] - f2[2] * f2[7]) + f1[4] * (f2[0] * f2[8] - f2[2] * f2[6]) - f1[5] * (f2[0] * f2[7] - f2[1] * f2[6]) +
           f1[6] * (f2[1] * f2[5] - f2[2] * f2[4]) - f1[7] * (f2[0] * f2[5] - f2[2] * f2[3]) + f1[8] * (f2[0] * f2[4] - f2[1] * f2[3]);
    t0 = f1[4] * f1[8] - f1[5] * f1[7]; t1 = f1[3] * f1[8] - f1[5] * f1[6]; t2 = f1[3] * f1[7] - f1[4] * f1[6];
    c[0] = f1[0] * t0 - f1[1] * t1 + f1[2] * t2;
    c[1] = f2[0] * t0 - f2[1] * t1 + f2[2] * t2 -
           f2[3] * (f1[1] * f1[8] - f1[2] * f1[7]) + f2[4] * (f1[0] * f1[8] - f1[2] * f1[6]) - f2[5] * (f1[0] * f1[7] - f1[1] * f1[6]) +
           f2[6] * (f1[1] * f1[5] - f1[2] * f1[4]) - f2[7] * (f1[0] * f1[5] - f1[2] * f1[3]) + f2[8] * (f1[0] * f1[4] - f1[1] * f1[3]);
    const int n = sgx_solve_cubic(c, r);
    if (n < 1 || n > 3) return n;
    for (int k = 0; k < n; k++, fmatrix += 9) {
        double lambda = r[k], mu = 1.;
        const double s = f1[8] * r[k] + f2[8];
        if (fabs(s) > DBL_EPSILON) { mu = 1. / s; lambda *= mu; fmatrix[8] = 1.; }
        else fmatrix[8] = 0.;
        for (int i = 0; i < 8; i++) fmatrix[i] = f1[i] * lambda + f2[i] * mu;
    }
    return n;
}

SGX_DEV float sgx_fm_error(const double *F, float m1x, float m1y, float m2x, float m2y)
{
    double a, b, c, d1, d2, s1, s2;
    a = F[0] * m1x + F[1] * m1y + F[2];
    b = F[3] * m1x + F[4] * m1y + F[5];
    c = F[6] * m1x + F[7] * m1y + F[8];
    s2 = 1. / (a * a + b * b);
    d2 = m2x * a + m2y * b + c;
    a = F[0] * m2x + F[3] * m2y + F[6];
    b = F[1] * m2x + F[4] * m2y + F[7];
    c = F[2] * m2x + F[5] * m2y + F[8];
    s1 = 1. / (a * a + b * b);
    d1 = m1x * a + m1y * b + c;
    const double e1 = d1 * d1 * s1, e2 = d2 * d2 * s2;
    return (float)(e1 < e2 ? e2 : e1);
}

SGX_DEV bool sgx_fm_collinear7(const float *p)
{
    const int i = 6;
    for (int j = 0; j < i; j++) {
        const double dx1 = p[2 * j] - p[2 * i], dy1 = p[2 * j + 1] - p[2 * i + 1];
        for (int k = 0; k < j; k++) {
            const double dx2 = p[2 * k] - p[2 * i], dy2 = p[2 * k + 1] - p[2 * i + 1];
            if (fabs(dx2 * dy1 - dy2 * dx1) <= FLT_EPSILON * (fabs(dx1) + fabs(dy1) + fabs(dx2) + fabs(dy2))) return true;
        }
    }
    return false;
}

SGX_DEV int sgx_ransac_update_num_iters(double p, double ep, int model_points, int max_iters)
{
    p = p > 0. ? p : 0.; p = p < 1. ? p : 1.;
    ep = ep > 0. ? ep : 0.; ep = ep < 1. ? ep : 1.;
    double num = 1. - p > DBL_MIN ? 1. - p : DBL_MIN;
    double denom = 1. - pow(1. - ep, (double)model_points);
    if (denom < DBL_MIN) return 0;
    num = log(num); denom = log(denom);
    return denom >= 0 || -num >= max_iters * (-denom) ? max_iters : (int)rint(num / denom);
}

struct SgxFmArgs {
    const uint8_t *keys; const int *n; int cap; const float *prev_xy;
    const int *pre_have; const float *pre_boxes; const int *pre_nboxes; int max_boxes;
    double threshold, confidence; int max_iters;
    double *F; int *ok; int *stats;
};

#ifndef SGX_FM_OCC
#define SGX_FM_OCC 2
#endif
SGX_KERNEL_OCC(256, SGX_FM_OCC) k_fm_ransac(SgxFmArgs A)
{
    SGX_DYN_LDS(lds_raw);
    const int f = (int)blockIdx.x, cap = A.cap;
    float *m1 = (float *)lds_raw, *m2 = m1 + 2 * cap;
    int *scan = (int *)(m2 + 2 * cap);
    uint8_t *flag = (uint8_t *)(scan + 256);
    SGX_LDS int s_total, s_count, s_done, s_niters, s_iter, s_maxgood, s_best_iter, s_best_root, s_attempts;
    SGX_LDS unsigned long long s_rng;
    SGX_LDS int g_idx[SGX_FM_CHUNK][7];
    SGX_LDS int g_nmodels[SGX_FM_CHUNK];
    SGX_LDS double g_model[SGX_FM_CHUNK][27];
    SGX_LDS int g_good[SGX_FM_CHUNK][3];
    SGX_LDS double g_work[SGX_FM_CHUNK][63];
    SGX_LDS double s_best[9];
    SGX_LDS float g_med[SGX_FM_CHUNK][3];
    SGX_LDS double s_minmed;
    const int N = min(A.n[f], cap), CH = (N + 255) / 256;
    const bool pre = A.pre_have && A.pre_have[f] && A.pre_boxes && A.pre_nboxes;

    SGX_THREADS_BEGIN(tid)
    int c = 0;
    for (int i = tid * CH; i < min(N, (tid + 1) * CH); i++) {
        uint8_t keep = 1;
        if (pre) {
            const float x = A.prev_xy[2 * ((size_t)f * cap + i)], y = A.prev_xy[2 * ((size_t)f * cap + i) + 1];
            const int nb = min(A.pre_nboxes[f], A.max_boxes);
            for (int q = 0; q < nb; q++) {
                const float *r = A.pre_boxes + 4 * ((size_t)f * A.max_boxes + q);
                if (x > r[0] && x < r[0] + r[2] && y > r[1] && y < r[1] + r[3]) { keep = 0; break; }
            }
        }
        flag[i] = keep; c += keep;
    }
    scan[tid] = c;
    if (tid == 0) { s_done = 0; s_niters = A.max_iters > 1 ? A.max_iters : 1; s_iter = 0; s_maxgood = 0; s_best_iter = 0; s_best_root = 0; s_attempts = 0; s_rng = ~0ull; }
    SGX_THREADS_END
    SGX_SYNC();
    SGX_THREADS_BEGIN(tid)
    sgx_block_exclusive_scan_i32(scan, 256, &s_total, tid);
    SGX_THREADS_END
    SGX_SYNC();
    const bool use_sel = pre && s_total > 20;
    SGX_THREADS_BEGIN(tid)
    int pos = use_sel ? scan[tid] : tid * CH;
    for (int i = tid * CH; i < min(N, (tid + 1) * CH); i++) {
        if (use_sel && !flag[i]) continue;
        const float *kp = (const float *)(A.keys + ((size_t)f * cap + i) * 28);
        m1[2 * pos] = kp[0]; m1[2 * pos + 1] = kp[1];
        m2[2 * pos] = A.prev_xy[2 * ((size_t)f * cap + i)]; m2[2 * pos + 1] = A.prev_xy[2 * ((size_t)f * cap + i) + 1];
        pos++;
    }
    if (tid == 0) s_count = use_sel ? s_total : N;
    SGX_THREADS_END
    SGX_SYNC();
    const int count = s_count;
    const float t = (float)(A.threshold * A.threshold);

    if (count < 7) {
        SGX_THREADS_BEGIN(tid)
        if (tid < 9) A.F[9 * (size_t)f + tid] = 0.;
        if (tid == 0) { A.ok[f] = 0; if (A.stats) { A.stats[4 * f] = 0; A.stats[4 * f + 1] = 0; A.stats[4 * f + 2] = 0; A.stats[4 * f + 3] = 0; } }
        SGX_THREADS_END
        return;
    }
    if (count == 7) {
        SGX_THREADS_BEGIN(tid)
        if (tid == 0) {
            const int k = sgx_fm_run7point(m1, m2, g_work[0], g_model[0]);
            for (int i = 0; i < 9; i++) A.F[9 * (size_t)f + i] = k > 0 ? g_model[0][i] : 0.;
            A.ok[f] = k > 0;
            if (A.stats) { A.stats[4 * f] = 0; A.stats[4 * f + 1] = 0; A.stats[4 * f + 2] = 0; A.stats[4 * f + 3] = 0; }
        }
        SGX_THREADS_END
        return;
    }

    const bool lmeds = count < 15;
    if (lmeds) {
        SGX_THREADS_BEGIN(tid)
        if (tid == 0) { const int ni = sgx_ransac_update_num_iters(A.confidence, 0.45, 7, 1000); s_niters = ni > 3 ? ni : 3; s_minmed = DBL_MAX; }
        SGX_THREADS_END
        SGX_SYNC();
    }
    for (int round = 0;; round++) {
        const int G = round == 0 && !lmeds ? 8 : SGX_FM_CHUNK;
        SGX_THREADS_BEGIN(tid)
        if (tid == 0) {
            unsigned long long st = s_rng;
            for (int gI = 0; gI < G; gI++)
                for (int i = 0; i < 7; i++) {
                    int idx_i, j;
                    for (;;) {
                        st = (unsigned long long)(unsigned)st * 4164903690ull + (unsigned)(st >> 32);
                        idx_i = (int)((unsigned)st % (unsigned)count);
                        for (j = 0; j < i; j++) if (idx_i == g_idx[gI][j]) break;
                        if (j == i) break;
                    }
                    g_idx[gI][i] = idx_i;
                }
            s_rng = st;
        }
        SGX_THREADS_END
        SGX_SYNC();
        SGX_THREADS_BEGIN(tid)
        if (tid < G) {
            float a[14], b[14];
            for (int i = 0; i < 7; i++) { const int id = g_idx[tid][i]; a[2 * i] = m1[2 * id]; a[2 * i + 1] = m1[2 * id + 1]; b[2 * i] = m2[2 * id]; b[2 * i + 1] = m2[2 * id + 1]; }
            int nm = -1;
            if (!sgx_fm_collinear7(a) && !sgx_fm_collinear7(b)) { nm = sgx_fm_run7point(a, b, g_work[tid], g_model[tid]); if (nm < 0 || nm > 3) nm = 0; }
            g_nmodels[tid] = nm;
            g_good[tid][0] = g_good[tid][1] = g_good[tid][2] = 0;
        }
        SGX_THREADS_END
        SGX_SYNC();
        if (lmeds) {
            SGX_THREADS_BEGIN(tid)
            if (tid < 3 * G) {
                const int gI = tid / 3, k = tid - 3 * gI;
                if (k < g_nmodels[gI]) {
                    double Fm[9]; float err[16];
                    for (int i = 0; i < 9; i++) Fm[i] = g_model[gI][9 * k + i];
                    for (int p = 0; p < count; p++) {
                        const float v = sgx_fm_error(Fm, m1[2 * p], m1[2 * p + 1], m2[2 * p], m2[2 * p + 1]);
                        int b = p - 1; while (b >= 0 && err[b] > v) { err[b + 1] = err[b]; b--; }
                        err[b + 1] = v;
                    }
                    g_med[gI][k] = err[count / 2];
                }
            }
            SGX_THREADS_END
            SGX_SYNC();
            SGX_THREADS_BEGIN(tid)
            if (tid == 0) {
                int iter = s_iter, attempts = s_attempts; const int niters = s_niters; double minmed = s_minmed;
                bool done = false;
                for (int gI = 0; gI < G && !done; gI++) {
                    if (iter >= niters) { done = true; break; }
                    if (g_nmodels[gI] < 0) { if (++attempts >= 10000) done = true; continue; }
                    attempts = 0;
                    for (int k = 0; k < g_nmodels[gI]; k++) {
                        const double med = (double)g_med[gI][k];
                        if (med < minmed) { minmed = med; for (int i = 0; i < 9; i++) s_best[i] = g_model[gI][9 * k + i]; s_best_iter = iter; s_best_root = k; }
                    }
                    iter++;
                }
                if (iter >= niters) done = true;
                s_iter = iter; s_attempts = attempts; s_minmed = minmed; s_done = done ? 1 : 0;
            }
            SGX_THREADS_END
            SGX_SYNC();
            if (s_done) break;
            continue;
        }
        for (int gI = 0; gI < G; gI++) {
            const int nm = g_nmodels[gI];
            for (int k = 0; k < nm; k++) {
                SGX_THREADS_BEGIN(tid)
                double Fm[9];
                for (int i = 0; i < 9; i++) Fm[i] = g_model[gI][9 * k + i];
                int cnt = 0;
                for (int p = tid; p < count; p += 256) cnt += sgx_fm_error(Fm, m1[2 * p], m1[2 * p + 1], m2[2 * p], m2[2 * p + 1]) <= t ? 1 : 0;
                if (cnt) sgx_atomic_add(&g_good[gI][k], cnt);
                SGX_THREADS_END
            }
        }
        SGX_SYNC();
        SGX_THREADS_BEGIN(tid)
        if (tid == 0) {
            int iter = s_iter, niters = s_niters, maxgood = s_maxgood, attempts = s_attempts;
            bool done = false;
            for (int gI = 0; gI < G && !done; gI++) {
                if (iter >= niters) { done = true; break; }
                if (g_nmodels[gI] < 0) {
                    if (++attempts >= 10000) done = true;
                    continue;
                }
                attempts = 0;
                for (int k = 0; k < g_nmodels[gI]; k++) {
                    const int good = g_good[gI][k];
                    if (good > (maxgood > 6 ? maxgood : 6)) {
                        for (int i = 0; i < 9; i++) s_best[i] = g_model[gI][9 * k + i];
                        maxgood = good; s_best_iter = iter; s_best_root = k;
                        niters = sgx_ransac_update_num_iters(A.confidence, (double)(count - good) / count, 7, niters);
                    }
                }
                iter++;
            }
            if (iter >= niters) done = true;
            s_iter = iter; s_niters = niters; s_maxgood = maxgood; s_attempts = attempts; s_done = done ? 1 : 0;
        }
        SGX_THREADS_END
        SGX_SYNC();
        if (s_done) break;
    }
    if (lmeds) {
        SGX_THREADS_BEGIN(tid)
        if (tid == 0) {
            int good = 0;
            if (s_minmed < DBL_MAX) {
                double sigma = 2.5 * 1.4826 * (1 + 5. / (count - 7)) * sqrt(s_minmed);
                if (sigma < 0.001) sigma = 0.001;
                const float ts = (float)(sigma * sigma);
                for (int p = 0; p < count; p++) good += sgx_fm_error(s_best, m1[2 * p], m1[2 * p + 1], m2[2 * p], m2[2 * p + 1]) <= ts ? 1 : 0;
            }
            s_maxgood = good >= 7 ? good : 0;
            if (A.stats) A.stats[4 * f + 3] = good;
        }
        SGX_THREADS_END
        SGX_SYNC();
    }
    SGX_THREADS_BEGIN(tid)
    const bool ok = s_maxgood > 0;
    if (tid < 9) A.F[9 * (size_t)f + tid] = ok ? s_best[tid] : 0.;
    if (tid == 0) {
        A.ok[f] = ok ? 1 : 0;
        if (A.stats) { A.stats[4 * f] = s_iter; A.stats[4 * f + 1] = s_best_iter; A.stats[4 * f + 2] = s_best_root; if (!lmeds) A.stats[4 * f + 3] = s_maxgood; }
    }
    SGX_THREADS_END
}
```

### sg_slam_amd/flow.py

```python
import ctypes as C
import numpy as np
from .capi import FlowConfig, _vp
from ._lib import load


class OpticalFlowLK:

    def __init__(self, width=640, height=480, max_batch=1, win_size=21, max_level=3, max_count=30, epsilon=0.01, lib=None):
        self.lib = lib if lib is not None else load()
        self.cfg = FlowConfig(width, height, max_batch, win_size, max_level, max_count, epsilon)
        h = C.c_void_p()
        self.lib.check(self.lib.dll.sgx_flow_create(C.byref(self.cfg), C.byref(h)), 'sgx_flow_create')
        self.h = h
        self.width, self.height, self.max_batch = width, height, max_batch
        self.levels = self.lib.dll.sgx_flow_levels(self.h)

    def close(self):
        if getattr(self, 'h', None):
            self.lib.dll.sgx_flow_destroy(self.h)
            self.h = None

    def __del__(self):
        try:
            self.close()
        except Exception:
            pass

    def reset(self):
        self.lib.check(self.lib.dll.sgx_flow_reset(self.h), 'sgx_flow_reset')

    def __call__(self, gray_from, gray_to, pts):
        a = np.ascontiguousarray(gray_from, np.uint8); b = np.ascontiguousarray(gray_to, np.uint8)
        assert a.shape == b.shape == (self.height, self.width)
        p = np.ascontiguousarray(pts, 'f4').reshape(-1, 2); n = len(p)
        out = np.zeros((max(n, 1), 2), 'f4'); st = np.zeros(max(n, 1), np.uint8)
        self.lib.check(self.lib.dll.sgx_flow_lk(self.h, _vp(a), _vp(b), self.width, _vp(p), n, _vp(out), _vp(st)), 'sgx_flow_lk')
        return out[:n], st[:n]

    def lk_batch_dev(self, d_gray, pitch, batch, d_keys, d_n, cap, d_prev_xy, d_status=None, stream=None):
        have = C.c_int32(0)
        self.lib.check(self.lib.dll.sgx_flow_lk_batch_dev(self.h, _vp(d_gray), pitch, batch, _vp(d_keys), _vp(d_n), cap, _vp(d_prev_xy), _vp(d_status),
                                                          C.byref(have), _vp(stream)), 'sgx_flow_lk_batch_dev')
        return bool(have.value)

    def debug_level(self, slot, frame, level):
        w, h = C.c_int32(), C.c_int32()
        self.lib.check(self.lib.tap('sgx_flow_debug_level_size')(self.h, level, C.byref(w), C.byref(h)))
        img = np.zeros((h.value, w.value), np.uint8)
        self.lib.check(self.lib.tap('sgx_flow_debug_read_level')(self.h, slot, frame, level, _vp(img)), 'flow debug_read_level')
        return img


def find_fundamental_mat(pts1, pts2, threshold=1.0, confidence=0.99, lib=None):
    lib = lib if lib is not None else load()
    a = np.ascontiguousarray(pts1, 'f4').reshape(-1, 2); b = np.ascontiguousarray(pts2, 'f4').reshape(-1, 2)
    assert len(a) == len(b)
    F = np.zeros(9, 'f8'); ok = np.zeros(1, 'i4'); stats = np.zeros(4, 'i4')
    lib.check(lib.dll.sgx_find_fundamental_mat(_vp(a), _vp(b), len(a), threshold, confidence, _vp(F), _vp(ok), _vp(stats)), 'sgx_find_fundamental_mat')
    return int(ok[0]), F.reshape(3, 3), stats


def fundamental_ransac_batch_dev(lib, batch, cap, d_keys, d_n, d_prev_xy, d_F, d_ok, d_stats=None, pre_have=None, pre_boxes=None, pre_nboxes=None, max_boxes=0,
                                 threshold=1.0, confidence=0.99, stream=None):
    lib.check(lib.dll.sgx_fundamental_ransac_batch_dev(batch, cap, _vp(d_keys), _vp(d_n), _vp(d_prev_xy), _vp(pre_have), _vp(pre_boxes), _vp(pre_nboxes), max_boxes,
                                                       threshold, confidence, _vp(d_F), _vp(d_ok), _vp(d_stats), _vp(stream)), 'sgx_fundamental_ransac_batch_dev')
```

Before: 29600.

## Precompute Scharr derivative planes per pyramid level for LK tracking

Adds a kernel that computes Scharr Ix/Iy derivative planes (int16, zero-padded apron) for pyramid levels at or above plane_min, once per frame while building the pyramid. The LK tracking kernels then read precomputed derivatives from these planes instead of recomputing 3x3 Scharr stencils per window sample. This trades per-keypoint recomputation for one extra full-image pass plus more global-memory traffic per sample (int16 planes vs u8). Level 0 still uses the old in-kernel derivative path by default.

```diff
diff --git a/include/sgx_debug.h b/include/sgx_debug.h
--- a/include/sgx_debug.h
+++ b/include/sgx_debug.h
@@ -19,6 +19,8 @@
 int sgx_det_debug_read_blob(sgx_det *h, const char *blob_name, int image, float *dst, int cap, int *n);
 int sgx_flow_debug_read_level(sgx_flow *h, int slot, int frame, int level, uint8_t *img);
 int sgx_flow_debug_level_size(const sgx_flow *h, int level, int32_t *w, int32_t *hgt);
+int sgx_flow_debug_read_deriv(sgx_flow *h, int frame, int level, int16_t *ixiy);
+int sgx_flow_debug_deriv_apron(sgx_flow *h, int frame, int level, int32_t *apron_x, int32_t *apron_y, int32_t *nonzero);
 int sgx_pnp_debug_betas(int which, const double *L, const double *rho, double *betas);
 int sgx_debug_corun_bf16(int blocks, int iters, int launches, void *stream);
 int sgx_det_debug_detection_output(sgx_det *h, const float *loc, const float *conf, int batch, sgx_det_result *results);
diff --git a/sg_slam_amd/capi.py b/sg_slam_amd/capi.py
--- a/sg_slam_amd/capi.py
+++ b/sg_slam_amd/capi.py
@@ -87,7 +87,7 @@
     'sgx_orb_debug_run_octree', 'sgx_pose_opt_debug_set_threads', 'sgx_ba_debug_set_solver', 'sgx_ba_debug_set_jobs', 'sgx_ba_debug_set_init', 'sgx_ba_debug_last_plan', 'sgx_det_debug_read_blob',
     'sgx_det_debug_detection_output', 'sgx_det_debug_continued', 'sgx_debug_flow_affine_batch_dev', 'sgx_det_debug_set_fusion', 'sgx_det_debug_set_legacy_kernels',
     'sgx_det_debug_set_block_fusion', 'sgx_det_debug_set_irb', 'sgx_det_debug_set_gemm', 'sgx_det_debug_time_ops', 'sgx_det_debug_run_step', 'sgx_flow_debug_read_level',
-    'sgx_flow_debug_level_size', 'sgx_debug_corun_bf16', 'sgx_pnp_debug_betas',
+    'sgx_flow_debug_level_size', 'sgx_debug_corun_bf16', 'sgx_pnp_debug_betas', 'sgx_flow_debug_read_deriv', 'sgx_flow_debug_deriv_apron',
 ]
 
 
@@ -246,6 +246,8 @@
             d.sgx_debug_corun_bf16.argtypes = [C.c_int, C.c_int, C.c_int, vp]
             d.sgx_pnp_debug_betas.argtypes = [C.c_int, vp, vp, vp]
             d.sgx_flow_debug_level_size.argtypes = [vp, C.c_int, C.POINTER(C.c_int32), C.POINTER(C.c_int32)]
+            d.sgx_flow_debug_read_deriv.argtypes = [vp, C.c_int, C.c_int, vp]
+            d.sgx_flow_debug_deriv_apron.argtypes = [vp, C.c_int, C.c_int] + [C.POINTER(C.c_int32)] * 3
 
     def tap(self, name):
         if not self.has_taps:
diff --git a/sg_slam_amd/csrc/sgx_flow.cpp b/sg_slam_amd/csrc/sgx_flow.cpp
--- a/sg_slam_amd/csrc/sgx_flow.cpp
+++ b/sg_slam_amd/csrc/sgx_flow.cpp
@@ -16,6 +16,7 @@
     sgx_flow_config cfg;
     SgxLkGeom g;
     uint8_t *img[2] = { nullptr, nullptr };
+    uint8_t *planes = nullptr;
     int cur = 0;
     int prev_batch = 0;
 };
@@ -46,6 +47,21 @@
     g.img_stride = (io + 15u + 64u) & ~15u;
     for (int s = 0; s < 2; s++)
         if (hipMalloc((void **)&h->img[s], (size_t)g.img_stride * cfg->max_batch) != hipSuccess) { sgx_flow_destroy(h); return SGX_ERR_NOMEM; }
+    const int pmin = sgx_getenv("SGX_LK_PLANE_MIN") ? atoi(sgx_getenv("SGX_LK_PLANE_MIN")) : 1;
+    g.plane_min = pmin < 0 ? 0 : pmin > g.nl ? g.nl : pmin;
+    unsigned po = 0;
+    for (int l = g.plane_min; l < g.nl; l++) {
+        g.ppitch[l] = (g.w[l] + 2 * SGX_LK_APRON_X + 7) & ~7;
+        g.pplane[l] = (unsigned)g.ppitch[l] * (unsigned)(g.h[l] + 2 * SGX_LK_APRON_Y) * 2u;
+        g.poff[l] = po + ((unsigned)SGX_LK_APRON_Y * (unsigned)g.ppitch[l] + SGX_LK_APRON_X) * 2u;
+        po += 2u * g.pplane[l];
+    }
+    g.plane_stride = po;
+    if (po) {
+        const size_t bytes = (size_t)po * cfg->max_batch;
+        if (hipMalloc((void **)&h->planes, bytes) != hipSuccess) { h->planes = nullptr; sgx_flow_destroy(h); return SGX_ERR_NOMEM; }
+        if (hipMemset(h->planes, 0, bytes) != hipSuccess || hipDeviceSynchronize() != hipSuccess) { sgx_flow_destroy(h); return SGX_ERR_DEVICE; }
+    }
     *out = h;
     return SGX_OK;
 }
@@ -54,13 +70,14 @@
 {
     if (!h) return;
     for (int s = 0; s < 2; s++) if (h->img[s]) (void)hipFree(h->img[s]);
+    if (h->planes) (void)hipFree(h->planes);
     delete h;
 }
 
 extern "C" int sgx_flow_reset(sgx_flow *h) { if (!h) return SGX_ERR_INVALID; h->prev_batch = 0; return SGX_OK; }
 extern "C" int sgx_flow_levels(const sgx_flow *h) { return h ? h->g.nl : SGX_ERR_INVALID; }
 
-static int build_pyramid(sgx_flow *h, int slot, const uint8_t *d_gray, int pitch, int batch, sgx_stream_t st)
+static int build_pyramid(sgx_flow *h, int slot, const uint8_t *d_gray, int pitch, int batch, bool with_planes, sgx_stream_t st)
 {
     const SgxLkGeom &g = h->g;
     uint8_t *base = h->img[slot];
@@ -70,6 +87,12 @@
     for (int l = 1; l < g.nl; l++)
         SGX_LAUNCH(k_lk_pyrdown, dim3(((g.pitch[l] >> 2) * g.h[l] + 255) / 256, batch), dim3(256), st, (const uint8_t *)(base + g.ioff[l - 1]), g.w[l - 1], g.h[l - 1], g.pitch[l - 1],
                    g.img_stride, base + g.ioff[l], g.w[l], g.h[l], g.pitch[l], g.img_stride, magic(g.pitch[l] >> 2));
+    if (with_planes && g.plane_min < g.nl) {
+        SgxLkMagic mg; memset(&mg, 0, sizeof mg);
+        for (int l = g.plane_min; l < g.nl; l++) mg.m[l] = magic(g.pitch[l] >> 2);
+        const int lp = g.plane_min;
+        SGX_LAUNCH(k_lk_deriv, dim3(((g.pitch[lp] >> 2) * g.h[lp] + 255) / 256, batch, g.nl - g.plane_min), dim3(256), st, g, mg, (const uint8_t *)base, h->planes);
+    }
     sgx_prof_end(SGX_K_LK_PYR, st);
     SGX_CHECK_HIP(hipGetLastError());
     return SGX_OK;
@@ -78,7 +101,7 @@
 static int track(sgx_flow *h, int cur_slot, int prev_slot, int batch, const sgx_keypoint *d_keys, const int32_t *d_n, int cap, float *d_prev_xy, uint8_t *d_status, sgx_stream_t st)
 {
     SgxLkArgs A;
-    A.cur_img = h->img[cur_slot]; A.prev_img = h->img[prev_slot];
+    A.cur_img = h->img[cur_slot]; A.prev_img = h->img[prev_slot]; A.planes = h->planes;
     A.keys = (const uint8_t *)d_keys; A.n = d_n; A.cap = cap; A.prev_xy = d_prev_xy; A.status = d_status;
     A.max_count = h->cfg.max_count > 100 ? 100 : h->cfg.max_count;
     double eps = h->cfg.epsilon > 10. ? 10. : h->cfg.epsilon;
@@ -106,7 +129,7 @@
     const int cur = h->cur, prev = cur ^ 1;
     const bool tracked = h->prev_batch == batch;
     if (tracked && (!d_keys || !d_n || !d_prev_xy || cap < 1)) return SGX_ERR_INVALID;
-    int rc = build_pyramid(h, cur, d_gray, pitch, batch, st);
+    int rc = build_pyramid(h, cur, d_gray, pitch, batch, tracked, st);
     if (rc != SGX_OK) return rc;
     if (tracked) { rc = track(h, cur, prev, batch, d_keys, d_n, cap, d_prev_xy, d_status, st); if (rc != SGX_OK) return rc; }
     if (have_prev) *have_prev = tracked ? 1 : 0;
@@ -128,8 +151,8 @@
     if ((rc = dI.put(0, pack.data(), pack.size())) != SGX_OK || (rc = dK.put(1, kp.data(), kp.size() * sizeof(sgx_keypoint))) != SGX_OK ||
         (rc = dN.put(2, &n, sizeof n)) != SGX_OK || (rc = dO.put(3, nullptr, (size_t)n * 8)) != SGX_OK || (rc = dS.put(4, nullptr, (size_t)n)) != SGX_OK) return rc;
     const int keep_cur = h->cur, keep_prev = h->prev_batch;
-    if ((rc = build_pyramid(h, 1, (const uint8_t *)dI.p, P, 1, 0)) != SGX_OK) return rc;
-    if ((rc = build_pyramid(h, 0, (const uint8_t *)dI.p + (size_t)P * H, P, 1, 0)) != SGX_OK) return rc;
+    if ((rc = build_pyramid(h, 1, (const uint8_t *)dI.p, P, 1, false, 0)) != SGX_OK) return rc;
+    if ((rc = build_pyramid(h, 0, (const uint8_t *)dI.p + (size_t)P * H, P, 1, true, 0)) != SGX_OK) return rc;
     if ((rc = track(h, 0, 1, 1, (const sgx_keypoint *)dK.p, (const int32_t *)dN.p, n, (float *)dO.p, (uint8_t *)dS.p, 0)) != SGX_OK) return rc;
     SGX_CHECK_HIP(hipMemcpy(next_pts, dO.p, (size_t)n * 8, hipMemcpyDeviceToHost));
     if (status) SGX_CHECK_HIP(hipMemcpy(status, dS.p, (size_t)n, hipMemcpyDeviceToHost));
@@ -154,6 +177,36 @@
 {
     if (!h || level < 0 || level >= h->g.nl || !w || !hh) return SGX_ERR_INVALID;
     *w = h->g.w[level]; *hh = h->g.h[level];
+    return SGX_OK;
+}
+
+SGX_TAP int sgx_flow_debug_read_deriv(sgx_flow *h, int frame, int level, int16_t *ixiy)
+{
+    if (!h || frame < 0 || frame >= h->cfg.max_batch || level < h->g.plane_min || level >= h->g.nl || !ixiy) return SGX_ERR_INVALID;
+    const SgxLkGeom &g = h->g;
+    SGX_CHECK_HIP(hipDeviceSynchronize());
+    const int pp = g.ppitch[level], w = g.w[level], hh = g.h[level];
+    std::vector<int16_t> t((size_t)g.pplane[level]);
+    SGX_CHECK_HIP(hipMemcpy(t.data(), h->planes + (size_t)frame * g.plane_stride + g.poff[level] - ((size_t)SGX_LK_APRON_Y * pp + SGX_LK_APRON_X) * 2, (size_t)g.pplane[level] * 2, hipMemcpyDeviceToHost));
+    const int16_t *ix = t.data() + (size_t)SGX_LK_APRON_Y * pp + SGX_LK_APRON_X, *iy = ix + g.pplane[level] / 2;
+    for (int y = 0; y < hh; y++) for (int x = 0; x < w; x++) { ixiy[((size_t)y * w + x) * 2] = ix[(size_t)y * pp + x]; ixiy[((size_t)y * w + x) * 2 + 1] = iy[(size_t)y * pp + x]; }
+    return SGX_OK;
+}
+SGX_TAP int sgx_flow_debug_deriv_apron(sgx_flow *h, int frame, int level, int32_t *apron_x, int32_t *apron_y, int32_t *nonzero)
+{
+    if (!h || frame < 0 || frame >= h->cfg.max_batch || level < h->g.plane_min || level >= h->g.nl || !nonzero) return SGX_ERR_INVALID;
+    const SgxLkGeom &g = h->g;
+    SGX_CHECK_HIP(hipDeviceSynchronize());
+    const int pp = g.ppitch[level], w = g.w[level], hh = g.h[level], rows = hh + 2 * SGX_LK_APRON_Y;
+    std::vector<int16_t> t((size_t)g.pplane[level]);
+    SGX_CHECK_HIP(hipMemcpy(t.data(), h->planes + (size_t)frame * g.plane_stride + g.poff[level] - ((size_t)SGX_LK_APRON_Y * pp + SGX_LK_APRON_X) * 2, (size_t)g.pplane[level] * 2, hipMemcpyDeviceToHost));
+    int32_t nz = 0;
+    for (int p = 0; p < 2; p++) for (int y = 0; y < rows; y++) for (int x = 0; x < pp; x++) {
+        const bool inside = y >= SGX_LK_APRON_Y && y < SGX_LK_APRON_Y + hh && x >= SGX_LK_APRON_X && x < SGX_LK_APRON_X + w;
+        if (!inside && t[((size_t)p * rows + y) * pp + x] != 0) nz++;
+    }
+    if (apron_x) *apron_x = SGX_LK_APRON_X; if (apron_y) *apron_y = SGX_LK_APRON_Y;
+    *nonzero = nz;
     return SGX_OK;
 }
 
diff --git a/sg_slam_amd/csrc/sgx_flow_kernels.h b/sg_slam_amd/csrc/sgx_flow_kernels.h
--- a/sg_slam_amd/csrc/sgx_flow_kernels.h
+++ b/sg_slam_amd/csrc/sgx_flow_kernels.h
@@ -12,7 +12,15 @@
     int w[SGX_LK_MAXL], h[SGX_LK_MAXL], pitch[SGX_LK_MAXL];
     unsigned ioff[SGX_LK_MAXL];
     unsigned img_stride;
+    int plane_min;
+    int ppitch[SGX_LK_MAXL];
+    unsigned poff[SGX_LK_MAXL];
+    unsigned pplane[SGX_LK_MAXL];
+    unsigned plane_stride;
 };
+#define SGX_LK_APRON_X 24
+#define SGX_LK_APRON_Y 22
+struct SgxLkMagic { unsigned m[SGX_LK_MAXL]; };
 
 SGX_DEV int sgx_reflect101(int p, int len)
 {
@@ -86,6 +94,76 @@
     SGX_THREADS_END
 }
 
+#ifndef SGX_EMU
+typedef short sgx_d16x2 __attribute__((ext_vector_type(2)));
+SGX_DEV sgx_d16x2 sgx_lk_widen2(uint32_t v, uint32_t sel) { return __builtin_bit_cast(sgx_d16x2, __builtin_amdgcn_perm(v, v, sel)); }
+SGX_DEV void sgx_lk_deriv4(const uint32_t (&lo)[3], const uint32_t (&hi)[3], uint32_t (&ix)[2], uint32_t (&iy)[2])
+{
+    const sgx_d16x2 c3 = { 3, 3 }, c10 = { 10, 10 };
+    sgx_d16x2 P[3][3];
+#pragma unroll
+    for (int j = 0; j < 3; j++) { P[j][0] = sgx_lk_widen2(lo[j], 0x0c010c00u); P[j][1] = sgx_lk_widen2(lo[j], 0x0c030c02u); P[j][2] = sgx_lk_widen2(hi[j], 0x0c010c00u); }
+    sgx_d16x2 S[3], D[3];
+#pragma unroll
+    for (int q = 0; q < 3; q++) { S[q] = (P[0][q] + P[2][q]) * c3 + P[1][q] * c10; D[q] = P[2][q] - P[0][q]; }
+#pragma unroll
+    for (int k = 0; k < 2; k++) {
+        const sgx_d16x2 mid = __builtin_bit_cast(sgx_d16x2, __builtin_amdgcn_alignbit(__builtin_bit_cast(uint32_t, D[k + 1]), __builtin_bit_cast(uint32_t, D[k]), 16));
+        ix[k] = __builtin_bit_cast(uint32_t, S[k + 1] - S[k]);
+        iy[k] = __builtin_bit_cast(uint32_t, (D[k] + D[k + 1]) * c3 + mid * c10);
+    }
+}
+#else
+static inline void sgx_lk_deriv4(const uint32_t (&lo)[3], const uint32_t (&hi)[3], uint32_t (&ix)[2], uint32_t (&iy)[2])
+{
+    int S[6], D[6];
+    for (int i = 0; i < 6; i++) {
+        int p[3];
+        for (int j = 0; j < 3; j++) p[j] = (int)(((i < 4 ? lo[j] : hi[j]) >> (8 * (i & 3))) & 255u);
+        S[i] = (p[0] + p[2]) * 3 + p[1] * 10; D[i] = p[2] - p[0];
+    }
+    for (int k = 0; k < 2; k++) {
+        int vx[2], vy[2];
+        for (int e = 0; e < 2; e++) { const int i = 2 * k + e + 1; vx[e] = S[i + 1] - S[i - 1]; vy[e] = (D[i - 1] + D[i + 1]) * 3 + D[i] * 10; }
+        ix[k] = ((uint32_t)vx[0] & 0xFFFFu) | ((uint32_t)vx[1] << 16); iy[k] = ((uint32_t)vy[0] & 0xFFFFu) | ((uint32_t)vy[1] << 16);
+    }
+}
+#endif
+SGX_KERNEL(256) k_lk_deriv(SgxLkGeom g, SgxLkMagic mg, const uint8_t *img, uint8_t *planes)
+{
+    SGX_THREADS_BEGIN(tid)
+    const int f = (int)blockIdx.y, l = g.plane_min + (int)blockIdx.z;
+    const int w = g.w[l], h = g.h[l], pitch = g.pitch[l], qw = pitch >> 2, q = (int)blockIdx.x * 256 + tid;
+    if (q < qw * h) {
+        const int y = (int)sgx_lk_udiv((unsigned)q, mg.m[l]), X = (q - y * qw) * 4;
+        const uint8_t *S = img + (size_t)f * g.img_stride + g.ioff[l];
+        const bool fast = X >= 4 && X + 4 <= w - 1;
+        uint32_t lo[3], hi[3];
+#pragma unroll
+        for (int j = 0; j < 3; j++) {
+            const uint8_t *row = S + (size_t)sgx_reflect101(y - 1 + j, h) * pitch;
+            if (fast) {
+                const uint32_t *r4 = (const uint32_t *)(row + X - 4);
+                const uint32_t a = r4[0], b = r4[1], c = r4[2];
+                lo[j] = (a >> 24) | (b << 8); hi[j] = (b >> 24) | (c << 8);
+            } else {
+                lo[j] = hi[j] = 0;
+#pragma unroll
+                for (int i = 0; i < 4; i++) { lo[j] |= (uint32_t)row[sgx_reflect101(X - 1 + i, w)] << (8 * i); hi[j] |= (uint32_t)row[sgx_reflect101(X + 3 + i, w)] << (8 * i); }
+            }
+        }
+        uint32_t ix[2], iy[2];
+        sgx_lk_deriv4(lo, hi, ix, iy);
+        uint8_t *px = planes + (size_t)f * g.plane_stride + g.poff[l] + ((size_t)y * g.ppitch[l] + X) * 2, *py = px + g.pplane[l];
+        if (X + 4 <= w) {
+            ((uint32_t *)px)[0] = ix[0]; ((uint32_t *)px)[1] = ix[1]; ((uint32_t *)py)[0] = iy[0]; ((uint32_t *)py)[1] = iy[1];
+        } else {
+            for (int i = 0; X + i < w; i++) { ((uint16_t *)px)[i] = (uint16_t)(ix[i >> 1] >> (16 * (i & 1))); ((uint16_t *)py)[i] = (uint16_t)(iy[i >> 1] >> (16 * (i & 1))); }
+        }
+    }
+    SGX_THREADS_END
+}
+
 struct SgxLkWeights { int w00, w01, w10, w11; };
 SGX_DEV SgxLkWeights sgx_lk_weights(float a, float b)
 {
@@ -111,6 +189,7 @@
 
 struct SgxLkArgs {
     const uint8_t *cur_img, *prev_img;
+    const uint8_t *planes;
     const uint8_t *keys; const int *n; int cap;
     float *prev_xy; uint8_t *status;
     int max_count; double eps2; float min_eig;
@@ -125,7 +204,7 @@
 
 #ifdef SGX_EMU
 static inline int sgx_lk_px(const uint8_t *I, int w, int h, int pitch, int x, int y) { return I[(size_t)sgx_reflect101(y, h) * pitch + sgx_reflect101(x, w)]; }
-static void sgx_lk_track_point(const SgxLkGeom &g, const uint8_t *I0, const uint8_t *J0, float kx, float ky, int max_count, double eps2, float min_eig,
+static void sgx_lk_track_point(const SgxLkGeom &g, const uint8_t *I0, const uint8_t *J0, const uint8_t *PL0, float kx, float ky, int max_count, double eps2, float min_eig,
                                float *ox, float *oy, uint8_t *ost)
 {
     const int W = SGX_LK_WIN; const float half = (W - 1) * 0.5f, FLT_SCALE = 1.f / (1 << 20);
@@ -134,6 +213,8 @@
     for (int level = g.nl - 1; level >= 0; level--) {
         const int w = g.w[level], h = g.h[level], pitch = g.pitch[level];
         const uint8_t *I = I0 + g.ioff[level], *J = J0 + g.ioff[level];
+        const bool planes = level >= g.plane_min;
+        const int16_t *PX = planes ? (const int16_t *)(PL0 + g.poff[level]) : nullptr, *PY = planes ? (const int16_t *)(PL0 + g.poff[level] + g.pplane[level]) : nullptr;
         const float sc = 1.0f / (float)(1 << level);
         float prevx = kx * sc, prevy = ky * sc, nextx, nexty;
         if (level == g.nl - 1) { nextx = prevx; nexty = prevy; } else { nextx = outx * 2.f; nexty = outy * 2.f; }
@@ -148,7 +229,8 @@
             for (int c = 0; c < 4; c++) {
                 const int gx = ipx + x + (c & 1), gy = ipy + y + (c >> 1);
                 pv[c] = sgx_lk_px(I, w, h, pitch, gx, gy);
-                if (gx < 0 || gy < 0 || gx >= w || gy >= h) { dx[c] = dy[c] = 0; }
+                if (planes) { const ptrdiff_t o = (ptrdiff_t)gy * g.ppitch[level] + gx; dx[c] = PX[o]; dy[c] = PY[o]; }
+                else if (gx < 0 || gy < 0 || gx >= w || gy >= h) { dx[c] = dy[c] = 0; }
                 else {
                     int t0[3], t1[3];
                     for (int q = 0; q < 3; q++) {
@@ -205,7 +287,7 @@
     if ((tid & 63) == 0 && kp < A.n[f] && kp < A.cap) {
         const float *kpt = (const float *)(A.keys + ((size_t)f * A.cap + kp) * 28);
         float ox, oy; uint8_t st;
-        sgx_lk_track_point(g, A.cur_img + (size_t)f * g.img_stride, A.prev_img + (size_t)f * g.img_stride, kpt[0], kpt[1], A.max_count, A.eps2, A.min_eig, &ox, &oy, &st);
+        sgx_lk_track_point(g, A.cur_img + (size_t)f * g.img_stride, A.prev_img + (size_t)f * g.img_stride, A.planes + (size_t)f * g.plane_stride, kpt[0], kpt[1], A.max_count, A.eps2, A.min_eig, &ox, &oy, &st);
         A.prev_xy[2 * ((size_t)f * A.cap + kp)] = ox; A.prev_xy[2 * ((size_t)f * A.cap + kp) + 1] = oy;
         if (A.status) A.status[(size_t)f * A.cap + kp] = st;
     }
@@ -230,6 +312,9 @@
 SGX_DEV int sgx_mul24(int a, int b) { return __mul24(a, b); }
 SGX_DEV int sgx_reflect1(int p, int len) { p = p < 0 ? -p : p; p = p >= len ? 2 * len - 2 - p : p; return min(max(p, 0), len - 1); }
 
+typedef __attribute__((address_space(3))) uint8_t sgx_lds_u8;
+typedef uint32_t sgx_u32x2 __attribute__((ext_vector_type(2)));
+typedef __attribute__((address_space(3))) sgx_u32x2 __attribute__((aligned(1))) sgx_lds_u32x2_u;
 typedef short sgx_i16x2 __attribute__((ext_vector_type(2)));
 typedef unsigned short sgx_u16x2 __attribute__((ext_vector_type(2)));
 SGX_DEV sgx_i16x2 sgx_as_i16x2(uint32_t v) { return __builtin_bit_cast(sgx_i16x2, v); }
@@ -273,6 +358,23 @@
         for (int p = 0; p < PASSES; p++) tile[(p * 7 + rl) * (SGX_LK_TILE_PITCH / 4) + cl] = v[p];
     }
     __builtin_amdgcn_fence(__ATOMIC_SEQ_CST, "wavefront"); __builtin_amdgcn_wave_barrier();
+}
+
+SGX_DEV void sgx_lk_segment_setup_planes(const uint32_t (&ia)[2], const uint32_t (&ib)[2], const uint32_t (&xa)[4], const uint32_t (&xb)[4], const uint32_t (&ya)[4], const uint32_t (&yb)[4],
+                                         sgx_i16x2 W0, sgx_i16x2 W1, int (&ivb)[7], uint32_t (&ixy)[7], int &s11, int &s12, int &s22)
+{
+#pragma unroll
+    for (int c = 0; c < 7; c++) {
+        const sgx_i16x2 pxa = (c & 1) ? sgx_lk_next(sgx_as_i16x2(xa[c >> 1]), sgx_as_i16x2(xa[(c >> 1) + 1])) : sgx_as_i16x2(xa[c >> 1]);
+        const sgx_i16x2 pxb = (c & 1) ? sgx_lk_next(sgx_as_i16x2(xb[c >> 1]), sgx_as_i16x2(xb[(c >> 1) + 1])) : sgx_as_i16x2(xb[c >> 1]);
+        const sgx_i16x2 pya = (c & 1) ? sgx_lk_next(sgx_as_i16x2(ya[c >> 1]), sgx_as_i16x2(ya[(c >> 1) + 1])) : sgx_as_i16x2(ya[c >> 1]);
+        const sgx_i16x2 pyb = (c & 1) ? sgx_lk_next(sgx_as_i16x2(yb[c >> 1]), sgx_as_i16x2(yb[(c >> 1) + 1])) : sgx_as_i16x2(yb[c >> 1]);
+        const int v = SGX_LK_DOT2(SGX_LK_PAIR(ib[1], ib[0], c, c + 1), W1, SGX_LK_DOT2(SGX_LK_PAIR(ia[1], ia[0], c, c + 1), W0, 256)) >> 9;
+        const int vx = SGX_LK_DOT2(pxb, W1, SGX_LK_DOT2(pxa, W0, 8192)) >> 14;
+        const int vy = SGX_LK_DOT2(pyb, W1, SGX_LK_DOT2(pya, W0, 8192)) >> 14;
+        ivb[c] = 256 - (v << 9); ixy[c] = ((uint32_t)vx & 0xFFFFu) | ((uint32_t)vy << 16);
+        s11 += sgx_mul24(vx, vx); s12 += sgx_mul24(vx, vy); s22 += sgx_mul24(vy, vy);
+    }
 }
 
 #ifdef SGX_DEBUG_TAPS
@@ -316,6 +418,23 @@
             const int gy0 = ipy + r, gx0 = ipx + s7;
             sgx_i16x2 P[4][5];
             const bool direct = ipx >= 1 && ipx + 25 < w && ipy >= 1 && ipy + 22 < h;
+            if (level >= g.plane_min) {
+                const int ppb = g.ppitch[level] * 2;
+                const uint8_t *px = A.planes + (size_t)f * g.plane_stride + g.poff[level] + (active ? gy0 * ppb + gx0 * 2 : 0);
+                const unsigned pyo = g.pplane[level];
+                uint32_t ia[2], ib[2], xa[4], xb[4], ya[4], yb[4]; uint32_t ixy[7];
+                if (direct) { const uint8_t *gb = I + (size_t)(active ? gy0 : ipy) * pitch + (active ? gx0 : ipx); __builtin_memcpy(ia, gb, 8); __builtin_memcpy(ib, gb + pitch, 8); }
+                else {
+                    const int tx = ((ipx - 1) >> 2) << 2, ty = ipy - 1;
+                    sgx_lk_stage<4>(tile, I, w, h, pitch, tx, ty, rl, cl);
+                    const uint8_t *tb = tile8 + lane_off + (ipx - 1 - tx) + SGX_LK_TILE_PITCH + 1;
+                    __builtin_memcpy(ia, tb, 8); __builtin_memcpy(ib, tb + SGX_LK_TILE_PITCH, 8);
+                }
+                __builtin_memcpy(xa, px, 16); __builtin_memcpy(xb, px + ppb, 16); __builtin_memcpy(ya, px + pyo, 16); __builtin_memcpy(yb, px + pyo + ppb, 16);
+                sgx_lk_segment_setup_planes(ia, ib, xa, xb, ya, yb, active ? W0 : sgx_as_i16x2(0u), active ? W1 : sgx_as_i16x2(0u), ivb, ixy, s11, s12, s22);
+#pragma unroll
+                for (int c = 0; c < 7; c++) { ix[c] = (int)(short)(ixy[c] & 0xFFFFu); iy[c] = (int)ixy[c] >> 16; }
+            } else {
             if (direct) {
                 const uint8_t *gb = I + (size_t)(active ? gy0 - 1 : ipy) * pitch + (active ? gx0 - 1 : ipx);
 #pragma unroll
@@ -375,6 +494,7 @@
                 const int vy = SGX_LK_DOT2(pyb, Wd1, SGX_LK_DOT2(pya, Wd0, 8192)) >> 14;
                 ivb[c] = 256 - (v << 9); ix[c] = vx; iy[c] = vy;
                 s11 += sgx_mul24(vx, vx); s12 += sgx_mul24(vx, vy); s22 += sgx_mul24(vy, vy);
+            }
             }
         }
         const float A11 = sgx_wave_sum_f32(s11) * FLT_SCALE, A12 = sgx_wave_sum_f32(s12) * FLT_SCALE, A22 = sgx_wave_sum_f32(s22) * FLT_SCALE;
@@ -559,6 +679,29 @@
                 if (act && !direct) sgx_lk_stage_row<28, LPK>(tile, I, w, h, pitch, tx, ty, l16);
                 __builtin_amdgcn_fence(__ATOMIC_SEQ_CST, "wavefront"); __builtin_amdgcn_wave_barrier();
             }
+            if (level >= g.plane_min) {
+                const uint8_t *PX = A.planes + (size_t)f * g.plane_stride + g.poff[level];
+                const int ppb = g.ppitch[level] * 2;
+                const unsigned pyo = g.pplane[level];
+#pragma unroll
+                for (int q = 0; q < SPL; q++) {
+                    const int gy0 = ipy + srow[q], gx0 = ipx + scol[q];
+                    uint32_t ia[2], ib[2], xa[4], xb[4], ya[4], yb[4];
+                    if (direct) { const uint8_t *gb = I + (size_t)gy0 * pitch + gx0; __builtin_memcpy(ia, gb, 8); __builtin_memcpy(ib, gb + pitch, 8); }
+                    else {
+                        const sgx_lds_u8 *tb = (const sgx_lds_u8 *)tile8 + soff[q] + (ipx - 1 - tx) + SGX_LK4_PITCH + 1;
+                        const sgx_u32x2 ta = *(const sgx_lds_u32x2_u *)tb, tc = *(const sgx_lds_u32x2_u *)(tb + SGX_LK4_PITCH);
+                        ia[0] = ta.x; ia[1] = ta.y; ib[0] = tc.x; ib[1] = tc.y;
+                    }
+                    const uint8_t *px = PX + (act ? gy0 * ppb + gx0 * 2 : 0);
+                    __builtin_memcpy(xa, px, 16); __builtin_memcpy(xb, px + ppb, 16);
+                    __builtin_memcpy(ya, px + pyo, 16); __builtin_memcpy(yb, px + pyo + ppb, 16);
+                    const bool on = act && !(q == SPL - 1 && idle3);
+                    const sgx_i16x2 Wq0 = on ? W0 : sgx_as_i16x2(0u), Wq1 = on ? W1 : sgx_as_i16x2(0u);
+                    sgx_lk_segment_setup_planes(ia, ib, xa, xb, ya, yb, Wq0, Wq1, ivb[q], ixy[q], s11, s12, s22);
+                    __builtin_amdgcn_sched_barrier(0);
+                }
+            } else {
 #pragma unroll
             for (int q = 0; q < SPL; q++) {
                 const int gy0 = ipy + srow[q], gx0 = ipx + scol[q];
@@ -588,6 +731,7 @@
                 const sgx_i16x2 Wq0 = on ? W0 : sgx_as_i16x2(0u), Wq1 = on ? W1 : sgx_as_i16x2(0u);
                 sgx_lk_segment_setup(P, Wq0, Wq1, whole, gx0, gy0, w, h, ivb[q], ixy[q], s11, s12, s22);
                 __builtin_amdgcn_sched_barrier(0);
+            }
             }
         }
         const float A11 = sgx_group_sum_f32<LPK>(s11) * FLT_SCALE, A12 = sgx_group_sum_f32<LPK>(s12) * FLT_SCALE, A22 = sgx_group_sum_f32<LPK>(s22) * FLT_SCALE;
@@ -663,7 +807,7 @@
     if (tid % (64 / KPW) == 0 && kp < A.n[f] && kp < A.cap) {
         const float *kpt = (const float *)(A.keys + ((size_t)f * A.cap + kp) * 28);
         float ox, oy; uint8_t st;
-        sgx_lk_track_point(g, A.cur_img + (size_t)f * g.img_stride, A.prev_img + (size_t)f * g.img_stride, kpt[0], kpt[1], A.max_count, A.eps2, A.min_eig, &ox, &oy, &st);
+        sgx_lk_track_point(g, A.cur_img + (size_t)f * g.img_stride, A.prev_img + (size_t)f * g.img_stride, A.planes + (size_t)f * g.plane_stride, kpt[0], kpt[1], A.max_count, A.eps2, A.min_eig, &ox, &oy, &st);
         A.prev_xy[2 * ((size_t)f * A.cap + kp)] = ox; A.prev_xy[2 * ((size_t)f * A.cap + kp) + 1] = oy;
         if (A.status) A.status[(size_t)f * A.cap + kp] = st;
     }
diff --git a/sg_slam_amd/flow.py b/sg_slam_amd/flow.py
--- a/sg_slam_amd/flow.py
+++ b/sg_slam_amd/flow.py
@@ -51,6 +51,19 @@
         return img
 
 
+    def debug_deriv(self, frame, level):
+        w, h = C.c_int32(), C.c_int32()
+        self.lib.check(self.lib.tap('sgx_flow_debug_level_size')(self.h, level, C.byref(w), C.byref(h)))
+        d = np.zeros((h.value, w.value, 2), np.int16)
+        self.lib.check(self.lib.tap('sgx_flow_debug_read_deriv')(self.h, frame, level, _vp(d)), 'flow debug_read_deriv')
+        return d
+
+    def debug_deriv_apron(self, frame, level):
+        ax, ay, nz = C.c_int32(), C.c_int32(), C.c_int32()
+        self.lib.check(self.lib.tap('sgx_flow_debug_deriv_apron')(self.h, frame, level, C.byref(ax), C.byref(ay), C.byref(nz)), 'flow debug_deriv_apron')
+        return ax.value, ay.value, nz.value
+
+
 def find_fundamental_mat(pts1, pts2, threshold=1.0, confidence=0.99, lib=None):
     lib = lib if lib is not None else load()
     a = np.ascontiguousarray(pts1, 'f4').reshape(-1, 2); b = np.ascontiguousarray(pts2, 'f4').reshape(-1, 2)
```

Result: no change. 29590, median of 2 (-0.0%).
